# freewym/espresso

Hardware: AMD Instinct MI355X
Metric: audio-hours/sec training (LibriSpeech Conformer-12 + CTC) (higher is better)
Workload: dtype bf16; 1 GPU; LibriSpeech 960h Conformer-12 + CTC update step, <=26000 frames & <=24 utts per GPU, V=5004, on-GPU fbank+CMVN+SpecAugment, dropout 0.1, clip 2.0, Adam; parallelism=dp1

## Files before the change

espresso_amd/csrc/conv_igemm.hip:

```cpp
#include <hip/hip_runtime.h>

#include "gemm_common.h"

namespace {

typedef const __attribute__((address_space(1))) void* gptr_t;
typedef __attribute__((address_space(3))) void* lptr_t;

struct ConvGatherArgs {
  const bf16_t* src;
  const bf16_t* W;
  bf16_t* out;
  const float* bias;
  double* stats;
  const bf16_t* zero;
  int RB, RT, RF;
  int ST, SF, SC;
  int at, af;
  int ntaps;
  int bt[9], bf[9], koff[9];
  int N;
  long ldw;
  int OT, OF, ot_mul, ot_add, of_mul, of_add;
};

template <int BN_>
__global__ __launch_bounds__(256, 2) void conv_gather_kernel(const ConvGatherArgs a) {
  constexpr int BM_ = 128, NST = 2;
  constexpr int NJ = BN_ / 32;
  constexpr int A_BYTES = BM_ * ROW_BYTES, STAGE = A_BYTES + BN_ * ROW_BYTES;
  constexpr int NA = BM_ / 32, NB = BN_ / 32;
  extern __shared__ __attribute__((aligned(16))) char dsm[];
  const int tid = threadIdx.x, lane = tid & 63, wave = tid >> 6;
  const int wm = wave >> 1, wcol = (wave & 1) * (BN_ / 2);
  const uint32_t M = (uint32_t)a.RB * a.RT * a.RF;
  const uint32_t m0 = blockIdx.x * BM_;
  const int cpt = a.SC / BK;
  const int nk = a.ntaps * cpt;

  int rowb[NA], rowt[NA], rowf[NA];
  int cs[NA];
#pragma unroll
  for (int i = 0; i < NA; ++i) {
    const int r = (wave + 4 * i) * 8 + (lane >> 3);
    cs[i] = (lane & 7) ^ (r & 7) ^ ((r >> 4) & 7);
    const uint32_t p = m0 + r;
    if (p < M) {
      const uint32_t q = p / (uint32_t)a.RF, b = q / (uint32_t)a.RT;
      const int rf = (int)(p - q * a.RF), rt = (int)(q - b * a.RT);
      rowb[i] = (int)b * a.ST;
      rowt[i] = rt * a.at;
      rowf[i] = rf * a.af;
    } else {
      rowb[i] = -1;
      rowt[i] = rowf[i] = 0;
    }
  }
  const bf16_t* bp[NB];
#pragma unroll
  for (int i = 0; i < NB; ++i) {
    const int r = (wave + 4 * i) * 8 + (lane >> 3);
    const int c = (lane & 7) ^ (r & 7) ^ ((r >> 4) & 7);
    bp[i] = a.W + (long)min(r, a.N - 1) * a.ldw + c * 8;
  }
  auto issue = [&](int stage, int kt) {
    const int tap = kt / cpt, chunk = kt - tap * cpt;
    const int dt = a.bt[tap], df = a.bf[tap];
    const long ko = a.koff[tap] + chunk * BK;
    char* base = dsm + stage * STAGE + wave * 1024;
#pragma unroll
    for (int i = 0; i < NA; ++i) {
      const int st = rowt[i] + dt, sf = rowf[i] + df;
      const bool ok = rowb[i] >= 0 && (unsigned)st < (unsigned)a.ST && (unsigned)sf < (unsigned)a.SF;
      const bf16_t* s = ok ? a.src + (((long)(rowb[i] + st)) * a.SF + sf) * a.SC + chunk * BK + cs[i] * 8 : a.zero + cs[i] * 8;
      __builtin_amdgcn_global_load_lds((gptr_t)s, (lptr_t)(base + i * 4096), 16, 0, 0);
    }
#pragma unroll
    for (int i = 0; i < NB; ++i)
      __builtin_amdgcn_global_load_lds((gptr_t)(bp[i] + ko), (lptr_t)(base + A_BYTES + i * 4096), 16, 0, 0);
  };

  f32x4_t acc[4][NJ];
#pragma unroll
  for (int i = 0; i < 4; ++i)
#pragma unroll
    for (int j = 0; j < NJ; ++j) acc[i][j] = (f32x4_t){0.f, 0.f, 0.f, 0.f};
  uint32_t a_off[2][4], b_off[2][NJ];
#pragma unroll
  for (int ks = 0; ks < 2; ++ks) {
#pragma unroll
    for (int i = 0; i < 4; ++i) a_off[ks][i] = lds_off(wm * 64 + i * 16 + (lane & 15), ks * 4 + (lane >> 4));
#pragma unroll
    for (int j = 0; j < NJ; ++j) b_off[ks][j] = A_BYTES + lds_off(wcol + j * 16 + (lane & 15), ks * 4 + (lane >> 4));
  }

  if (nk > 0) issue(0, 0);
  int stage = 0;
  for (int kt = 0; kt < nk; ++kt) {
    asm volatile("s_waitcnt vmcnt(0)" ::: "memory");
    __builtin_amdgcn_s_barrier();
    if (kt + 1 < nk) issue(stage ^ 1, kt + 1);
    const char* st = dsm + stage * STAGE;
#pragma unroll
    for (int ks = 0; ks < 2; ++ks) {
      bf16x8_t af[4], bfr[NJ];
#pragma unroll
      for (int i = 0; i < 4; ++i) af[i] = *reinterpret_cast<const bf16x8_t*>(st + a_off[ks][i]);
#pragma unroll
      for (int j = 0; j < NJ; ++j) bfr[j] = *reinterpret_cast<const bf16x8_t*>(st + b_off[ks][j]);
#pragma unroll
      for (int i = 0; i < 4; ++i)
#pragma unroll
        for (int j = 0; j < NJ; ++j)
          acc[i][j] = __builtin_amdgcn_mfma_f32_16x16x32_bf16(
              __builtin_bit_cast(__attribute__((ext_vector_type(8))) __bf16, af[i]),
              __builtin_bit_cast(__attribute__((ext_vector_type(8))) __bf16, bfr[j]), acc[i][j], 0, 0, 0);
    }
    stage ^= 1;
  }

  constexpr int CG = BN_ / 8;
  constexpr int RL = 256 / CG;
  float* sC = reinterpret_cast<float*>(dsm);
  const int cg = tid % CG, rlane = tid / CG;
  float bias8[8], s8[8], q8[8];
#pragma unroll
  for (int e = 0; e < 8; ++e) {
    bias8[e] = a.bias ? a.bias[cg * 8 + e] : 0.f;
    s8[e] = q8[e] = 0.f;
  }
#pragma unroll 1
  for (int half = 0; half < 2; ++half) {
    __syncthreads();
    if (wm == half) {
#pragma unroll
      for (int i = 0; i < 4; ++i)
#pragma unroll
        for (int j = 0; j < NJ; ++j)
#pragma unroll
          for (int r = 0; r < 4; ++r) sC[(i * 16 + (lane >> 4) * 4 + r) * BN_ + wcol + j * 16 + (lane & 15)] = acc[i][j][r];
    }
    __syncthreads();
#pragma unroll 1
    for (int pass = 0; pass < 64 / RL; ++pass) {
      const int rl = pass * RL + rlane;
      const uint32_t p = m0 + half * 64 + rl;
      if (p < M) {
        const uint32_t q = p / (uint32_t)a.RF, b = q / (uint32_t)a.RT;
        const int rf = (int)(p - q * a.RF), rt = (int)(q - b * a.RT);
        const long orow = ((long)b * a.OT + (long)rt * a.ot_mul + a.ot_add) * a.OF + (long)rf * a.of_mul + a.of_add;
        const float4 x0 = *reinterpret_cast<const float4*>(sC + rl * BN_ + cg * 8);
        const float4 x1 = *reinterpret_cast<const float4*>(sC + rl * BN_ + cg * 8 + 4);
        float v[8] = {x0.x, x0.y, x0.z, x0.w, x1.x, x1.y, x1.z, x1.w};
#pragma unroll
        for (int e = 0; e < 8; ++e) v[e] += bias8[e];
        uint4 u;
        u.x = pack_bf2(v[0], v[1]); u.y = pack_bf2(v[2], v[3]); u.z = pack_bf2(v[4], v[5]); u.w = pack_bf2(v[6], v[7]);
        *reinterpret_cast<uint4*>(a.out + orow * a.N + cg * 8) = u;
        if (a.stats) {
          const uint32_t w[4] = {u.x, u.y, u.z, u.w};
#pragma unroll
          for (int e = 0; e < 4; ++e) {
            const float lo = __uint_as_float(w[e] << 16), hi = __uint_as_float(w[e] & 0xffff0000u);
            s8[2 * e] += lo; q8[2 * e] += lo * lo;
            s8[2 * e + 1] += hi; q8[2 * e + 1] += hi * hi;
          }
        }
      }
    }
  }
  if (a.stats) {
    __syncthreads();
    float* red = reinterpret_cast<float*>(dsm);
#pragma unroll
    for (int e = 0; e < 8; ++e) {
      red[(rlane * 2 + 0) * BN_ + cg * 8 + e] = s8[e];
      red[(rlane * 2 + 1) * BN_ + cg * 8 + e] = q8[e];
    }
    __syncthreads();
    if (tid < 2 * BN_) {
      const int which = tid / BN_, c = tid - which * BN_;
      float t = 0.f;
      for (int r = 0; r < RL; ++r) t += red[(r * 2 + which) * BN_ + c];
      atomicAdd(a.stats + which * a.N + c, (double)t);
    }
  }
}

const bf16_t* zero_line(hipStream_t stream) {
  static bf16_t* z = nullptr;
  if (!z) {
    if (hipMalloc(&z, 256) != hipSuccess) return nullptr;
    if (hipMemsetAsync(z, 0, 256, stream) != hipSuccess) return nullptr;
    hipStreamSynchronize(stream);
  }
  return z;
}

template <int BN_>
int launch_gather(const ConvGatherArgs& a, hipStream_t stream) {
  constexpr int bytes = 2 * (128 + BN_) * ROW_BYTES;
  static bool attr_ok = hipFuncSetAttribute(reinterpret_cast<const void*>(&conv_gather_kernel<BN_>),
                                            hipFuncAttributeMaxDynamicSharedMemorySize, bytes) == hipSuccess;
  if (!attr_ok) return -1;
  const long M = (long)a.RB * a.RT * a.RF;
  if (M <= 0) return 0;
  if (M >= (1L << 31) - 128) return -1;
  hipLaunchKernelGGL((conv_gather_kernel<BN_>), dim3((unsigned)((M + 127) / 128)), dim3(256), bytes, stream, a);
  return EA_CHECK_LAUNCH();
}


struct ConvWgradArgs {
  const bf16_t* X;
  const bf16_t* dZ;
  float* slab;
  const bf16_t* zero;
  int RB, RT, RF, ST, SF, Cin, Cout;
  int at, af, ntaps;
  int bt[9], bf[9];
  int chunks_per_wg;
  int ablate;
};

__device__ __forceinline__ int tr_sw(int r) { return (r & 3) ^ ((r >> 3) & 1); }
__device__ __forceinline__ void ds_read_tr16_x8(const uint32_t (&ad)[8], uint2 (&o)[8]) {
  asm volatile(
      "ds_read_b64_tr_b16 %0, %8\n\tds_read_b64_tr_b16 %1, %9\n\tds_read_b64_tr_b16 %2, %10\n\tds_read_b64_tr_b16 %3, %11\n\t"
      "ds_read_b64_tr_b16 %4, %12\n\tds_read_b64_tr_b16 %5, %13\n\tds_read_b64_tr_b16 %6, %14\n\tds_read_b64_tr_b16 %7, %15\n\t"
      "s_waitcnt lgkmcnt(0)"
      : "=&v"(o[0]), "=&v"(o[1]), "=&v"(o[2]), "=&v"(o[3]), "=&v"(o[4]), "=&v"(o[5]), "=&v"(o[6]), "=&v"(o[7])
      : "v"(ad[0]), "v"(ad[1]), "v"(ad[2]), "v"(ad[3]), "v"(ad[4]), "v"(ad[5]), "v"(ad[6]), "v"(ad[7])
      : "memory");
}

template <int DEPTH, int NT>
__global__ __launch_bounds__(256, NT == 9 ? 2 : 4) void conv_wgrad_kernel(const ConvWgradArgs a) {
  constexpr int TILE = 64 * ROW_BYTES;
  constexpr int NBUF = DEPTH == 1 ? 2 : 4;
  static_assert(DEPTH >= 1 && DEPTH <= 3 && (NT == 9 || NT == 3), "ring of two / four X tiles");
  const int tap0 = NT == 9 ? 0 : (int)(blockIdx.z % 3) * 3;
  const int zsplit = NT == 9 ? (int)blockIdx.z : (int)(blockIdx.z / 3);
  __shared__ __attribute__((aligned(16))) char lds[(2 + NBUF) * TILE];
  const int tid = threadIdx.x, lane = tid & 63, wave = tid >> 6;
  const int wr = wave >> 1, wc = wave & 1;
  const int co0 = blockIdx.x * 64, ci0 = blockIdx.y * 64;
  const long M = (long)a.RB * a.RT * a.RF;
  const long chunk0 = (long)zsplit * a.chunks_per_wg;
  long nch = (M + 63) / 64 - chunk0;
  if (nch > a.chunks_per_wg) nch = a.chunks_per_wg;
  if (nch < 0) nch = 0;

  f32x4_t acc[NT][2][2];
#pragma unroll
  for (int t = 0; t < NT; ++t)
#pragma unroll
    for (int i = 0; i < 2; ++i)
#pragma unroll
      for (int j = 0; j < 2; ++j) acc[t][i][j] = (f32x4_t){0.f, 0.f, 0.f, 0.f};

  int rr[2], cs[2];
#pragma unroll
  for (int i = 0; i < 2; ++i) {
    rr[i] = (wave + 4 * i) * 8 + (lane >> 3);
    cs[i] = (lane & 7) ^ (tr_sw(rr[i]) << 1);
  }
  int rowb[2], rowt[2], rowf[2];
  long rowp[2];
  auto decode = [&](long ch) {
#pragma unroll
    for (int i = 0; i < 2; ++i) {
      const long p = (chunk0 + ch) * 64 + rr[i];
      rowp[i] = p;
      if (p < M) {
        const uint32_t q = (uint32_t)p / (uint32_t)a.RF, b = q / (uint32_t)a.RT;
        rowb[i] = (int)b * a.ST;
        rowt[i] = (int)(q - b * a.RT) * a.at;
        rowf[i] = (int)((uint32_t)p - q * a.RF) * a.af;
      } else {
        rowb[i] = -1;
        rowt[i] = rowf[i] = 0;
      }
    }
  };
  auto issue_A = [&](int abuf) {
#pragma unroll
    for (int i = 0; i < 2; ++i) {
      const bf16_t* s = rowb[i] >= 0 ? a.dZ + rowp[i] * a.Cout + co0 + cs[i] * 8 : a.zero + cs[i] * 8;
      __builtin_amdgcn_global_load_lds((gptr_t)s, (lptr_t)(lds + abuf * TILE + (wave + 4 * i) * 1024), 16, 0, 0);
    }
  };
  auto issue_B = [&](int buf, int tap) {
#pragma unroll
    for (int i = 0; i < 2; ++i) {
      const int st = rowt[i] + a.bt[tap0 + tap], sf = rowf[i] + a.bf[tap0 + tap];
      const bool ok = rowb[i] >= 0 && (unsigned)st < (unsigned)a.ST && (unsigned)sf < (unsigned)a.SF;
      const bf16_t* s = ok ? a.X + (((long)(rowb[i] + st)) * a.SF + sf) * a.Cin + ci0 + cs[i] * 8 : a.zero + cs[i] * 8;
      __builtin_amdgcn_global_load_lds((gptr_t)s, (lptr_t)(lds + (2 + buf) * TILE + (wave + 4 * i) * 1024), 16, 0, 0);
    }
  };
  const uint32_t lds0 = (uint32_t)(uintptr_t)lds;
  auto read_frags = [&](int tile_off, int c0, uint4 (&fr)[2][2]) {
    const int g = lane >> 4, i = lane & 15;
    uint32_t ad[8];
    uint2 o[8];
#pragma unroll
    for (int ks = 0; ks < 2; ++ks)
#pragma unroll
      for (int t = 0; t < 2; ++t)
#pragma unroll
        for (int h = 0; h < 2; ++h) {
          const int r = ks * 32 + 8 * g + (i >> 2) + 4 * h;
          const int chunk = (c0 >> 4) + t;
          ad[(ks * 2 + t) * 2 + h] = lds0 + tile_off + r * ROW_BYTES + ((chunk ^ tr_sw(r)) << 5) + (i & 3) * 8;
        }
    ds_read_tr16_x8(ad, o);
#pragma unroll
    for (int ks = 0; ks < 2; ++ks)
#pragma unroll
      for (int t = 0; t < 2; ++t) fr[ks][t] = make_uint4(o[(ks * 2 + t) * 2].x, o[(ks * 2 + t) * 2].y, o[(ks * 2 + t) * 2 + 1].x, o[(ks * 2 + t) * 2 + 1].y);
  };

  const int nsteps = (int)nch * NT;
  int is = 0, itap = 0;
  long ich = 0;
  auto issue_next = [&]() {
    if (is >= nsteps) return;
    if (!(a.ablate & 2) || is < DEPTH) {
      if (itap == 0) {
        decode(ich);
        issue_A((int)(ich & 1));
      }
      issue_B(is & (NBUF - 1), itap);
    }
    ++is;
    if (++itap == NT) { itap = 0; ++ich; }
  };
#pragma unroll
  for (int d = 0; d < DEPTH; ++d) issue_next();
  uint4 fa[2][2];
  long ch = 0;
  int tap = 0;
  for (int s = 0; s < nsteps; ++s) {
    const int tap1 = tap + 1 == NT ? 0 : tap + 1, tap2 = tap1 + 1 == NT ? 0 : tap1 + 1;
    int pend = 0;
    if (DEPTH >= 2 && s + 1 < nsteps) pend += 2 + (tap1 == 0 ? 2 : 0);
    if (DEPTH >= 3 && s + 2 < nsteps) pend += 2 + (tap2 == 0 ? 2 : 0);
    if (pend >= 8) asm volatile("s_waitcnt vmcnt(8)" ::: "memory");
    else if (pend == 6) asm volatile("s_waitcnt vmcnt(6)" ::: "memory");
    else if (pend == 4) asm volatile("s_waitcnt vmcnt(4)" ::: "memory");
    else if (pend == 2) asm volatile("s_waitcnt vmcnt(2)" ::: "memory");
    else asm volatile("s_waitcnt vmcnt(0)" ::: "memory");
    if (!(a.ablate & 8)) __builtin_amdgcn_s_barrier();
    uint4 fb[2][2];
    if (!(a.ablate & 4) || s == 0) {
      if (tap == 0) read_frags((int)(ch & 1) * TILE, wr * 32, fa);
      read_frags((2 + (s & (NBUF - 1))) * TILE, wc * 32, fb);
    } else {
      fb[0][0] = fb[0][1] = fb[1][0] = fb[1][1] = fa[0][0];
    }
    __builtin_amdgcn_sched_barrier(0);
    issue_next();
    if (!(a.ablate & 1)) {
#pragma unroll
    for (int t = 0; t < NT; ++t) {
      if (t == tap) {
#pragma unroll
        for (int ks = 0; ks < 2; ++ks)
#pragma unroll
          for (int i = 0; i < 2; ++i)
#pragma unroll
            for (int j = 0; j < 2; ++j)
              acc[t][i][j] = __builtin_amdgcn_mfma_f32_16x16x32_bf16(
                  __builtin_bit_cast(__attribute__((ext_vector_type(8))) __bf16, fa[ks][i]),
                  __builtin_bit_cast(__attribute__((ext_vector_type(8))) __bf16, fb[ks][j]), acc[t][i][j], 0, 0, 0);
      }
    }
    } else {
      acc[0][0][0][0] += __uint_as_float(fb[0][0].x) + __uint_as_float(fb[1][1].y);
    }
    tap = tap1;
    if (tap1 == 0) ++ch;
  }

  float* out = a.slab + (long)zsplit * a.Cout * a.ntaps * a.Cin;
#pragma unroll
  for (int t = 0; t < NT; ++t) {
    {
#pragma unroll
      for (int i = 0; i < 2; ++i)
#pragma unroll
        for (int j = 0; j < 2; ++j)
#pragma unroll
          for (int r = 0; r < 4; ++r) {
            const int co = co0 + wr * 32 + i * 16 + (lane >> 4) * 4 + r, ci = ci0 + wc * 32 + j * 16 + (lane & 15);
            out[((long)co * a.ntaps + tap0 + t) * a.Cin + ci] = acc[t][i][j][r];
          }
    }
  }
}

__global__ __launch_bounds__(256) void conv_wgrad_reduce_kernel(const float* __restrict__ slab, float* __restrict__ dW, long n, int nsplit,
                                                                int cin = 0) {
  const int zper = (nsplit + gridDim.y - 1) / gridDim.y;
  const int z0 = blockIdx.y * zper, z1 = min(nsplit, z0 + zper);
  const long i = ((long)blockIdx.x * 256 + threadIdx.x) * 4;
  if (i >= n || z0 >= z1) return;
  float4 s = *reinterpret_cast<const float4*>(slab + (long)z0 * n + i);
  for (int z = z0 + 1; z < z1; ++z) {
    const float4 x = *reinterpret_cast<const float4*>(slab + (long)z * n + i);
    s.x += x.x; s.y += x.y; s.z += x.z; s.w += x.w;
  }
  if (cin > 0) {
    const long ct = i / cin;
    const int ci = (int)(i - ct * cin), tap = (int)(ct % 9);
    const long co = ct / 9;
    float* d = dW + (co * cin + ci) * 9 + tap;
    const float v[4] = {s.x, s.y, s.z, s.w};
#pragma unroll
    for (int e = 0; e < 4; ++e) {
      if (gridDim.y == 1) d[9 * e] += v[e];
      else atomicAdd(d + 9 * e, v[e]);
    }
    return;
  }
  if (gridDim.y == 1) {
    float4 d = *reinterpret_cast<const float4*>(dW + i);
    d.x += s.x; d.y += s.y; d.z += s.z; d.w += s.w;
    *reinterpret_cast<float4*>(dW + i) = d;
  } else {
    atomicAdd(dW + i, s.x); atomicAdd(dW + i + 1, s.y); atomicAdd(dW + i + 2, s.z); atomicAdd(dW + i + 3, s.w);
  }
}

static int wgrad_split(long M, int Cin, int Cout) {
  const long chunks = (M + 63) / 64;
  const int blocks = (Cin / 64) * (Cout / 64);
  static const long target = [] { const char* e = getenv("EA_CONV_WGRAD_WGS"); const long v = e ? atol(e) : 0; return v > 0 ? v : 256L; }();
  long nsplit = (target + blocks - 1) / blocks;
  if (nsplit > chunks / 8) nsplit = chunks / 8;
  if (nsplit < 1) nsplit = 1;
  return (int)nsplit;
}

}

extern "C" int ea_conv3x3_fwd(const void* X, const void* W, const float* bias, void* Z, double* stats, int B, int T, int F,
                              int Cin, int Cout, int sy, int sx, hipStream_t stream) {
  if (B <= 0 || T <= 0 || F <= 0) return 0;
  if (Cin % 64 || (Cout != 64 && Cout != 128) || sy < 1 || sx < 1) return -2;
  ConvGatherArgs a;
  a.src = (const bf16_t*)X; a.W = (const bf16_t*)W; a.out = (bf16_t*)Z; a.bias = bias; a.stats = stats;
  a.zero = zero_line(stream);
  if (!a.zero) return -1;
  const int To = (T - 1) / sy + 1, Fo = (F - 1) / sx + 1;
  a.RB = B; a.RT = To; a.RF = Fo;
  a.ST = T; a.SF = F; a.SC = Cin;
  a.at = sy; a.af = sx;
  a.ntaps = 9;
  for (int ky = 0; ky < 3; ++ky)
    for (int kx = 0; kx < 3; ++kx) {
      const int t = ky * 3 + kx;
      a.bt[t] = ky - 1; a.bf[t] = kx - 1; a.koff[t] = t * Cin;
    }
  a.N = Cout; a.ldw = 9L * Cin;
  a.OT = To; a.OF = Fo; a.ot_mul = 1; a.ot_add = 0; a.of_mul = 1; a.of_add = 0;
  return Cout == 128 ? launch_gather<128>(a, stream) : launch_gather<64>(a, stream);
}

extern "C" int ea_conv3x3_dgrad(const void* dZ, const void* Wd, void* dX, int B, int T, int F, int Cin, int Cout, int sy, int sx,
                                hipStream_t stream) {
  if (B <= 0 || T <= 0 || F <= 0) return 0;
  if (Cout % 64 || (Cin != 64 && Cin != 128) || sy < 1 || sx < 1 || sy > 2 || sx > 2) return -2;
  const int To = (T - 1) / sy + 1, Fo = (F - 1) / sx + 1;
  const bf16_t* zero = zero_line(stream);
  if (!zero) return -1;
  for (int pt = 0; pt < sy; ++pt)
    for (int pf = 0; pf < sx; ++pf) {
      ConvGatherArgs a;
      a.src = (const bf16_t*)dZ; a.W = (const bf16_t*)Wd; a.out = (bf16_t*)dX; a.bias = nullptr; a.stats = nullptr; a.zero = zero;
      a.RB = B; a.RT = (T - pt + sy - 1) / sy; a.RF = (F - pf + sx - 1) / sx;
      a.ST = To; a.SF = Fo; a.SC = Cout;
      a.at = 1; a.af = 1;
      a.ntaps = 0;
      for (int ky = 0; ky < 3; ++ky) {
        if ((pt + 1 - ky) % sy) continue;
        for (int kx = 0; kx < 3; ++kx) {
          if ((pf + 1 - kx) % sx) continue;
          const int t = a.ntaps++;
          a.bt[t] = (pt + 1 - ky) / sy; a.bf[t] = (pf + 1 - kx) / sx; a.koff[t] = (ky * 3 + kx) * Cout;
        }
      }
      a.N = Cin; a.ldw = 9L * Cout;
      a.OT = T; a.OF = F; a.ot_mul = sy; a.ot_add = pt; a.of_mul = sx; a.of_add = pf;
      if (a.RT <= 0 || a.RF <= 0) continue;
      if (a.ntaps == 0) return -2;
      const int rc = Cin == 128 ? launch_gather<128>(a, stream) : launch_gather<64>(a, stream);
      if (rc) return rc;
    }
  return 0;
}

extern "C" long ea_conv3x3_wgrad_workspace_bytes(int B, int T, int F, int Cin, int Cout, int sy, int sx) {
  const int To = (T - 1) / sy + 1, Fo = (F - 1) / sx + 1;
  return (long)wgrad_split((long)B * To * Fo, Cin, Cout) * Cout * 9 * Cin * (long)sizeof(float);
}

static int conv3x3_wgrad_impl(const void* X, const void* dZ, float* dW, void* workspace, int B, int T, int F, int Cin, int Cout,
                              int sy, int sx, int param_layout, hipStream_t stream);
extern "C" int ea_conv3x3_wgrad(const void* X, const void* dZ, float* dW, void* workspace, int B, int T, int F, int Cin, int Cout,
                                int sy, int sx, hipStream_t stream) {
  return conv3x3_wgrad_impl(X, dZ, dW, workspace, B, T, F, Cin, Cout, sy, sx, 0, stream);
}
extern "C" int ea_conv3x3_wgrad_param_layout(const void* X, const void* dZ, float* dW, void* workspace, int B, int T, int F, int Cin,
                                             int Cout, int sy, int sx, hipStream_t stream) {
  return conv3x3_wgrad_impl(X, dZ, dW, workspace, B, T, F, Cin, Cout, sy, sx, 1, stream);
}
static int conv3x3_wgrad_impl(const void* X, const void* dZ, float* dW, void* workspace, int B, int T, int F, int Cin, int Cout,
                              int sy, int sx, int param_layout, hipStream_t stream) {
  if (B <= 0 || T <= 0 || F <= 0) return 0;
  if (Cin % 64 || Cout % 64 || sy < 1 || sx < 1 || !workspace) return -2;
  ConvWgradArgs a;
  a.X = (const bf16_t*)X; a.dZ = (const bf16_t*)dZ; a.slab = (float*)workspace;
  a.zero = zero_line(stream);
  if (!a.zero) return -1;
  const int To = (T - 1) / sy + 1, Fo = (F - 1) / sx + 1;
  a.RB = B; a.RT = To; a.RF = Fo; a.ST = T; a.SF = F; a.Cin = Cin; a.Cout = Cout;
  a.at = sy; a.af = sx; a.ntaps = 9;
  for (int ky = 0; ky < 3; ++ky)
    for (int kx = 0; kx < 3; ++kx) { a.bt[ky * 3 + kx] = ky - 1; a.bf[ky * 3 + kx] = kx - 1; }
  const long M = (long)B * To * Fo;
  if (M >= (1L << 31) - 128) return -2;
  const int nsplit = wgrad_split(M, Cin, Cout);
  const long chunks = (M + 63) / 64;
  a.chunks_per_wg = (int)((chunks + nsplit - 1) / nsplit);
  static const int ablate = [] { const char* e = getenv("EA_CONVW_ABLATE"); return e ? atoi(e) : 0; }();
  a.ablate = ablate;
  static const int depth_env = [] { const char* e = getenv("EA_CONV_WGRAD_DEPTH"); return e ? atoi(e) : 0; }();
  const int depth = depth_env ? depth_env : (Cout <= 64 ? 3 : 1);
  static const int taps_env = [] { const char* e = getenv("EA_CONV_WGRAD_TAPS"); return e ? atoi(e) : 0; }();
  const int taps = taps_env == 3 || taps_env == 9 ? taps_env : 3;
  if (taps == 3) {
    hipLaunchKernelGGL((conv_wgrad_kernel<1, 3>), dim3(Cout / 64, Cin / 64, nsplit * 3), dim3(256), 0, stream, a);
  } else if (depth == 1) hipLaunchKernelGGL((conv_wgrad_kernel<1, 9>), dim3(Cout / 64, Cin / 64, nsplit), dim3(256), 0, stream, a);
  else if (depth == 2) hipLaunchKernelGGL((conv_wgrad_kernel<2, 9>), dim3(Cout / 64, Cin / 64, nsplit), dim3(256), 0, stream, a);
  else hipLaunchKernelGGL((conv_wgrad_kernel<3, 9>), dim3(Cout / 64, Cin / 64, nsplit), dim3(256), 0, stream, a);
  const long n = (long)Cout * 9 * Cin;
  const long blocks = (n / 4 + 255) / 256;
  int zg = (int)(1024 / blocks);
  if (zg > nsplit / 4) zg = nsplit / 4;
  if (zg < 1) zg = 1;
  hipLaunchKernelGGL(conv_wgrad_reduce_kernel, dim3((unsigned)blocks, zg), dim3(256), 0, stream, (const float*)workspace, dW, n, nsplit,
                     param_layout ? Cin : 0);
  return EA_CHECK_LAUNCH();
}
```

espresso_amd/csrc/convmodule.hip:

```cpp
#include "common.h"
#include "espresso_amd.h"

namespace {

constexpr int KMAX = 31;

__device__ __forceinline__ float sigmoid_f(float x) { return __builtin_amdgcn_rcpf(1.f + __expf(-x)); }

constexpr int CT = 64, TTILE = 64, TPT = TTILE / 4;

template <int KW>
__global__ __launch_bounds__(256) void glu_dwconv_fwd_kernel(const bf16_t* __restrict__ Y,
                                                             const float* __restrict__ w,
                                                             bf16_t* __restrict__ U, bf16_t* __restrict__ Z,
                                                             double* __restrict__ stats, int T, int C) {
  constexpr int PAD = (KW - 1) / 2, ROWS = TTILE + KW - 1;
  __shared__ __attribute__((aligned(16))) float su[ROWS][CT];
  __shared__ float sred[2][4][CT];
  const int c0 = blockIdx.x * CT, t0 = blockIdx.y * TTILE, b = blockIdx.z;
  const long rowbase = (long)b * T;
  if ((C & 7) == 0 && c0 + CT <= C) {
    bf16_t (*sub)[CT] = reinterpret_cast<bf16_t (*)[CT]>(&su[0][0]);
    bf16_t (*sz)[CT] = reinterpret_cast<bf16_t (*)[CT]>(&su[0][0]) + ROWS;
    constexpr int NCH = (ROWS * (CT / 8) + 255) / 256;
// ... 19 lines not shown
        const int tin = t0 - PAD + row;
        const uint32_t aw[4] = {va[k].x, va[k].y, va[k].z, va[k].w}, gw[4] = {vg[k].x, vg[k].y, vg[k].z, vg[k].w};
        uint32_t pk[4];
#pragma unroll
        for (int e = 0; e < 4; ++e)
          pk[e] = pack_bf2(__uint_as_float(aw[e] << 16) * sigmoid_f(__uint_as_float(gw[e] << 16)),
                           __uint_as_float(aw[e] & 0xffff0000u) * sigmoid_f(__uint_as_float(gw[e] & 0xffff0000u)));
        const bool inside = tin >= 0 && tin < T;
        const uint4 u4 = inside ? make_uint4(pk[0], pk[1], pk[2], pk[3]) : make_uint4(0, 0, 0, 0);
        if (inside && row >= PAD && row < PAD + TTILE) *reinterpret_cast<uint4*>(U + (rowbase + tin) * C + c0 + c8) = u4;
        *reinterpret_cast<uint4*>(&sub[row][c8]) = u4;
      }
    }
    __syncthreads();
    float acc[TPT];
#pragma unroll
    for (int j = 0; j < TPT; ++j) acc[j] = 0.f;
#pragma unroll
    for (int r = 0; r < TPT + KW - 1; ++r) {
      const float x = bf2f(sub[grp * TPT + r][cl]);
#pragma unroll
      for (int j = 0; j < TPT; ++j)
        if (r - j >= 0 && r - j < KW) acc[j] += wk[r - j] * x;
    }
    float s = 0.f, q = 0.f;
#pragma unroll
    for (int j = 0; j < TPT; ++j) {
      const int tout = t0 + grp * TPT + j;
      const bf16_t zb = f2bf(acc[j]);
      sz[grp * TPT + j][cl] = zb;
      if (tout < T) {
        const float z = bf2f(zb);
        s += z;
        q += z * z;
      }
    }
    if (stats) {
      sred[0][grp][cl] = s;
      sred[1][grp][cl] = q;
    }
    __syncthreads();
#pragma unroll
    for (int k = 0; k < 2; ++k) {
      const int i = threadIdx.x + 256 * k;
      const int r = i >> 3, c8 = (i & 7) * 8;
      if (t0 + r < T) *reinterpret_cast<uint4*>(Z + (rowbase + t0 + r) * C + c0 + c8) = *reinterpret_cast<const uint4*>(&sz[r][c8]);
    }
    if (stats && threadIdx.x < CT) {
      const int x = threadIdx.x;
      atomicAdd(stats + c0 + x, (double)(sred[0][0][x] + sred[0][1][x] + sred[0][2][x] + sred[0][3][x]));
      atomicAdd(stats + C + c0 + x, (double)(sred[1][0][x] + sred[1][1][x] + sred[1][2][x] + sred[1][3][x]));
    }
    return;
  }
  const bool vec = (C & 7) == 0;
  for (int i = threadIdx.x; i < ROWS * (CT / 8); i += 256) {
    const int row = i / (CT / 8), c8 = (i % (CT / 8)) * 8;
    const int tin = t0 - PAD + row;
    float u[8];
#pragma unroll
    for (int e = 0; e < 8; ++e) u[e] = 0.f;
    if (tin >= 0 && tin < T && c0 + c8 < C) {
      const bf16_t* yr = Y + (rowbase + tin) * (2L * C) + c0 + c8;
      uint32_t pk[4] = {0, 0, 0, 0};
      if (vec && c0 + c8 + 8 <= C) {
        const uint4 av = *reinterpret_cast<const uint4*>(yr);
        const uint4 gv = *reinterpret_cast<const uint4*>(yr + C);
        const uint32_t aw[4] = {av.x, av.y, av.z, av.w}, gw[4] = {gv.x, gv.y, gv.z, gv.w};
#pragma unroll
        for (int e = 0; e < 4; ++e)
          pk[e] = pack_bf2(__uint_as_float(aw[e] << 16) * sigmoid_f(__uint_as_float(gw[e] << 16)),
                           __uint_as_float(aw[e] & 0xffff0000u) * sigmoid_f(__uint_as_float(gw[e] & 0xffff0000u)));
        if (row >= PAD && row < PAD + TTILE)
          *reinterpret_cast<uint4*>(U + (rowbase + tin) * C + c0 + c8) = make_uint4(pk[0], pk[1], pk[2], pk[3]);
      } else {
        for (int e = 0; e < 8; ++e) {
          if (c0 + c8 + e >= C) break;
          const bf16_t ub = f2bf(bf2f(yr[e]) * sigmoid_f(bf2f(yr[C + e])));
          if (row >= PAD && row < PAD + TTILE) U[(rowbase + tin) * C + c0 + c8 + e] = ub;
          pk[e >> 1] |= (uint32_t)ub << (16 * (e & 1));
        }
      }
#pragma unroll
      for (int e = 0; e < 4; ++e) {
        u[2 * e] = __uint_as_float(pk[e] << 16);
        u[2 * e + 1] = __uint_as_float(pk[e] & 0xffff0000u);
      }
    }
    *reinterpret_cast<float4*>(&su[row][c8]) = make_float4(u[0], u[1], u[2], u[3]);
    *reinterpret_cast<float4*>(&su[row][c8 + 4]) = make_float4(u[4], u[5], u[6], u[7]);
  }
  const int cl = threadIdx.x & (CT - 1), grp = threadIdx.x >> 6;
  const int c = c0 + cl;
  float wk[KW];
#pragma unroll
  for (int k = 0; k < KW; ++k) wk[k] = c < C ? w[(long)c * KW + k] : 0.f;
  __syncthreads();
  float acc[TPT];
#pragma unroll
  for (int j = 0; j < TPT; ++j) acc[j] = 0.f;
#pragma unroll
  for (int r = 0; r < TPT + KW - 1; ++r) {
    const float x = su[grp * TPT + r][cl];
#pragma unroll
    for (int j = 0; j < TPT; ++j)
      if (r - j >= 0 && r - j < KW) acc[j] += wk[r - j] * x;
  }
  float s = 0.f, q = 0.f;
#pragma unroll
  for (int j = 0; j < TPT; ++j) {
    const int tout = t0 + grp * TPT + j;
    if (tout < T && c < C) {
      const bf16_t zb = f2bf(acc[j]);
      Z[(rowbase + tout) * C + c] = zb;
      const float z = bf2f(zb);
      s += z;
      q += z * z;
    }
  }
  if (stats) {
    sred[0][grp][cl] = s;
    sred[1][grp][cl] = q;
    __syncthreads();
    if (threadIdx.x < CT && c0 + threadIdx.x < C) {
      const int x = threadIdx.x;
      atomicAdd(stats + c0 + x, (double)(sred[0][0][x] + sred[0][1][x] + sred[0][2][x] + sred[0][3][x]));
      atomicAdd(stats + C + c0 + x, (double)(sred[1][0][x] + sred[1][1][x] + sred[1][2][x] + sred[1][3][x]));
    }
  }
}

__global__ void bn_finalize_kernel(const double* __restrict__ stats, float* __restrict__ mean_rstd,
                                   float* __restrict__ running_mean, float* __restrict__ running_var,
                                   int C, float n, float eps, float momentum) {
  const int c = blockIdx.x * blockDim.x + threadIdx.x;
  if (c >= C) return;
  const float mean = (float)(stats[c] / (double)n);
  float var = (float)(stats[C + c] / (double)n - (stats[c] / (double)n) * (stats[c] / (double)n));
  var = fmaxf(var, 0.f);
  mean_rstd[c] = mean;
  mean_rstd[C + c] = rsqrtf(var + eps);
  if (running_mean) {
    running_mean[c] = (1.f - momentum) * running_mean[c] + momentum * mean;
    const float unb = n > 1.f ? var * n / (n - 1.f) : var;
    running_var[c] = (1.f - momentum) * running_var[c] + momentum * unb;
  }
}
__global__ void bn_from_running_kernel(const float* __restrict__ running_mean, const float* __restrict__ running_var,
                                       float* __restrict__ mean_rstd, int C, float eps) {
  const int c = blockIdx.x * blockDim.x + threadIdx.x;
  if (c >= C) return;
  mean_rstd[c] = running_mean[c];
  mean_rstd[C + c] = rsqrtf(running_var[c] + eps);
}

__global__ __launch_bounds__(256) void bn_act_fwd_kernel(const bf16_t* __restrict__ Z, const float* __restrict__ mean_rstd,
                                                         const float* __restrict__ gamma, const float* __restrict__ beta,
                                                         bf16_t* __restrict__ Hout, long M, int C, int act) {
  const int nch = C >> 3;
  const long total = M * nch;
  const long stride = (long)gridDim.x * blockDim.x;
  const int ch = (int)(((long)blockIdx.x * blockDim.x + threadIdx.x) % nch);
  float sc[8], sh[8];
#pragma unroll
  for (int e = 0; e < 8; ++e) {
    const int c = ch * 8 + e;
    sc[e] = mean_rstd[C + c] * gamma[c];
    sh[e] = beta[c] - mean_rstd[c] * sc[e];
  }
  for (long i = (long)blockIdx.x * blockDim.x + threadIdx.x; i < total; i += stride) {
    const long m = i / nch;
    const uint4 u = *reinterpret_cast<const uint4*>(Z + m * C + ch * 8);
    const uint32_t wv[4] = {u.x, u.y, u.z, u.w};
    float o[8];
#pragma unroll
    for (int e = 0; e < 8; ++e) {
      const float z = (e & 1) ? __uint_as_float(wv[e >> 1] & 0xffff0000u) : __uint_as_float(wv[e >> 1] << 16);
      const float y = z * sc[e] + sh[e];
      o[e] = act == 2 ? silu_f(y) : (act == 1 ? fmaxf(y, 0.f) : y);
    }
    uint4 r;
    r.x = pack_bf2(o[0], o[1]); r.y = pack_bf2(o[2], o[3]); r.z = pack_bf2(o[4], o[5]); r.w = pack_bf2(o[6], o[7]);
    *reinterpret_cast<uint4*>(Hout + m * C + ch * 8) = r;
  }
}

__global__ __launch_bounds__(256) void bn_act_fwd_stats_kernel(const bf16_t* __restrict__ Z, const double* __restrict__ stats,
                                                               float* __restrict__ mean_rstd, float* __restrict__ running_mean,
                                                               float* __restrict__ running_var, const float* __restrict__ gamma,
                                                               const float* __restrict__ beta, bf16_t* __restrict__ Hout, long M,
                                                               int C, int act, float n, float eps, float momentum,
                                                               double* __restrict__ zero_next, int zero_n) {
  extern __shared__ float s_scsh[];
  const int nch = C >> 3;
  const long total = M * nch;
  const long stride = (long)gridDim.x * blockDim.x;
  const long gtid = (long)blockIdx.x * blockDim.x + threadIdx.x;
  const double inv_n = 1.0 / (double)n;
  for (int c = threadIdx.x; c < C; c += 256) {
    const double m1 = stats[c] * inv_n;
    const float mean = (float)m1;
    float var = (float)(stats[C + c] * inv_n - m1 * m1);
    var = fmaxf(var, 0.f);
    const float rstd = rsqrtf(var + eps);
    const float scv = rstd * gamma[c];
    s_scsh[c] = scv;
    s_scsh[C + c] = beta[c] - mean * scv;
    if (blockIdx.x == 0) {
      mean_rstd[c] = mean;
      mean_rstd[C + c] = rstd;
      if (running_mean) {
        running_mean[c] = (1.f - momentum) * running_mean[c] + momentum * mean;
        const float unb = n > 1.f ? var * n / (n - 1.f) : var;
        running_var[c] = (1.f - momentum) * running_var[c] + momentum * unb;
      }
    }
  }
  __syncthreads();
  const int ch = (int)(gtid % nch);
  float sc[8], sh[8];
#pragma unroll
  for (int e = 0; e < 8; ++e) {
    sc[e] = s_scsh[ch * 8 + e];
    sh[e] = s_scsh[C + ch * 8 + e];
  }
  for (long i = gtid; i < total; i += stride) {
    const long m = i / nch;
    const uint4 u = *reinterpret_cast<const uint4*>(Z + m * C + ch * 8);
    const uint32_t wv[4] = {u.x, u.y, u.z, u.w};
    float o[8];
#pragma unroll
    for (int e = 0; e < 8; ++e) {
      const float z = (e & 1) ? __uint_as_float(wv[e >> 1] & 0xffff0000u) : __uint_as_float(wv[e >> 1] << 16);
      const float y = z * sc[e] + sh[e];
      o[e] = act == 2 ? silu_f(y) : (act == 1 ? fmaxf(y, 0.f) : y);
    }
    uint4 r;
    r.x = pack_bf2(o[0], o[1]); r.y = pack_bf2(o[2], o[3]); r.z = pack_bf2(o[4], o[5]); r.w = pack_bf2(o[6], o[7]);
    *reinterpret_cast<uint4*>(Hout + m * C + ch * 8) = r;
  }
  if (zero_next)
    for (long i = gtid; i < zero_n; i += stride) zero_next[i] = 0.0;
}

__global__ __launch_bounds__(256) void bn_act_bwd_reduce_kernel(const bf16_t* __restrict__ Z, const bf16_t* __restrict__ dH,
                                                                const float* __restrict__ mean_rstd,
                                                                const float* __restrict__ gamma, const float* __restrict__ beta,
                                                                float* __restrict__ red, long M, int C, int act,
                                                                int rows_per_block, int TCH) {
  extern __shared__ float sm[];
  const int nch = C >> 3;
  const int cx = threadIdx.x % TCH, ry = threadIdx.x / TCH, lanes = 256 / TCH;
  const int ch = blockIdx.x * TCH + cx;
  const long r0 = (long)blockIdx.y * rows_per_block;
  const long r1 = min(M, r0 + rows_per_block);
  float sa[8], sb[8];
#pragma unroll
  for (int e = 0; e < 8; ++e) sa[e] = sb[e] = 0.f;
  if (ch < nch) {
    float mu[8], rs[8], ga[8], be[8];
#pragma unroll
    for (int e = 0; e < 8; ++e) {
      const int c = ch * 8 + e;
      mu[e] = mean_rstd[c]; rs[e] = mean_rstd[C + c]; ga[e] = gamma[c]; be[e] = beta[c];
    }
    auto accum = [&](const uint4& uz, const uint4& ud) {
      const uint32_t wz[4] = {uz.x, uz.y, uz.z, uz.w}, wd[4] = {ud.x, ud.y, ud.z, ud.w};
#pragma unroll
      for (int e = 0; e < 8; ++e) {
        const float z = (e & 1) ? __uint_as_float(wz[e >> 1] & 0xffff0000u) : __uint_as_float(wz[e >> 1] << 16);
        float d = (e & 1) ? __uint_as_float(wd[e >> 1] & 0xffff0000u) : __uint_as_float(wd[e >> 1] << 16);
        const float xh = (z - mu[e]) * rs[e];
        const float y = xh * ga[e] + be[e];
        d *= act == 2 ? dsilu_f(y) : (act == 1 ? (y > 0.f ? 1.f : 0.f) : 1.f);
        sa[e] += d;
        sb[e] += d * xh;
      }
    };
    constexpr int R = 4;
    long m = r0 + ry;
    for (; m + (long)(R - 1) * lanes < r1; m += (long)R * lanes) {
      uint4 uz[R], ud[R];
#pragma unroll
      for (int r = 0; r < R; ++r) {
        uz[r] = *reinterpret_cast<const uint4*>(Z + (m + (long)r * lanes) * C + ch * 8);
        ud[r] = *reinterpret_cast<const uint4*>(dH + (m + (long)r * lanes) * C + ch * 8);
      }
#pragma unroll
      for (int r = 0; r < R; ++r) accum(uz[r], ud[r]);
    }
    for (; m < r1; m += lanes) {
      const uint4 uz = *reinterpret_cast<const uint4*>(Z + m * C + ch * 8);
      const uint4 ud = *reinterpret_cast<const uint4*>(dH + m * C + ch * 8);
      accum(uz, ud);
    }
  }
  float* mine = sm + ((long)ry * TCH + cx) * 16;
#pragma unroll
  for (int e = 0; e < 8; ++e) { mine[e] = sa[e]; mine[8 + e] = sb[e]; }
  __syncthreads();
  for (int o = threadIdx.x; o < TCH * 16; o += 256) {
    const int cxo = o / 16, e = o % 16;
    const int cho = blockIdx.x * TCH + cxo;
    if (cho >= nch) continue;
    float a = 0.f;
    for (int r = 0; r < lanes; ++r) a += sm[((long)r * TCH + cxo) * 16 + e];
// ... 233 lines not shown
  const int cl = threadIdx.x & (CT - 1), grp = threadIdx.x >> 6;
  float acc[KG];
#pragma unroll
  for (int k = 0; k < KG; ++k) acc[k] = 0.f;
  const int tbeg = blockIdx.y * tiles_per_block * TTILE, tend = min(T, tbeg + tiles_per_block * TTILE);
  for (int t0 = tbeg; t0 < tend; t0 += TTILE) {
    __syncthreads();
    const bool c_ok = (C & 7) == 0;
    for (int i = threadIdx.x; i < (ROWS + KG) * (CT / 8); i += 256) {
      const int row = i / (CT / 8), c8 = (i % (CT / 8)) * 8;
      const int tin = t0 - PAD + row;
      float u[8];
#pragma unroll
      for (int e = 0; e < 8; ++e) u[e] = 0.f;
      if (row < ROWS && tin >= 0 && tin < T) {
        const bf16_t* src = U + (rowbase + tin) * C + c0 + c8;
        if (c_ok && c0 + c8 + 8 <= C) {
          const uint4 v = *reinterpret_cast<const uint4*>(src);
          const uint32_t w[4] = {v.x, v.y, v.z, v.w};
#pragma unroll
          for (int e = 0; e < 4; ++e) {
            u[2 * e] = __uint_as_float(w[e] << 16);
            u[2 * e + 1] = __uint_as_float(w[e] & 0xffff0000u);
          }
        } else {
          for (int e = 0; e < 8; ++e)
            if (c0 + c8 + e < C) u[e] = bf2f(src[e]);
        }
      }
      *reinterpret_cast<float4*>(&sU[row][c8]) = make_float4(u[0], u[1], u[2], u[3]);
      *reinterpret_cast<float4*>(&sU[row][c8 + 4]) = make_float4(u[4], u[5], u[6], u[7]);
    }
    for (int i = threadIdx.x; i < TTILE * (CT / 8); i += 256) {
      const int row = i / (CT / 8), c8 = (i % (CT / 8)) * 8;
      const int t = t0 + row;
      float d[8];
#pragma unroll
      for (int e = 0; e < 8; ++e) d[e] = 0.f;
      if (t < T) {
        const bf16_t* src = dZ + (rowbase + t) * C + c0 + c8;
        if (c_ok && c0 + c8 + 8 <= C) {
          const uint4 v = *reinterpret_cast<const uint4*>(src);
          const uint32_t w[4] = {v.x, v.y, v.z, v.w};
#pragma unroll
          for (int e = 0; e < 4; ++e) {
            d[2 * e] = __uint_as_float(w[e] << 16);
            d[2 * e + 1] = __uint_as_float(w[e] & 0xffff0000u);
          }
        } else {
          for (int e = 0; e < 8; ++e)
            if (c0 + c8 + e < C) d[e] = bf2f(src[e]);
        }
      }
      *reinterpret_cast<float4*>(&sD[row][c8]) = make_float4(d[0], d[1], d[2], d[3]);
      *reinterpret_cast<float4*>(&sD[row][c8 + 4]) = make_float4(d[4], d[5], d[6], d[7]);
    }
    __syncthreads();
    float x[KG];
#pragma unroll
    for (int kk = 0; kk < KG - 1; ++kk) x[kk + 1] = sU[grp * KG + kk][cl];
#pragma unroll
    for (int tt = 0; tt < TTILE; ++tt) {
#pragma unroll
      for (int kk = 0; kk < KG - 1; ++kk) x[kk] = x[kk + 1];
      x[KG - 1] = sU[tt + grp * KG + KG - 1][cl];
      const float d = sD[tt][cl];
#pragma unroll
      for (int kk = 0; kk < KG; ++kk) acc[kk] += d * x[kk];
    }
  }
  const int c = c0 + cl;
  if (c < C) {
    float* out = part + (((long)b * gridDim.y + blockIdx.y) * C + c) * KW;
#pragma unroll
    for (int kk = 0; kk < KG; ++kk)
      if (grp * KG + kk < KW) out[grp * KG + kk] = acc[kk];
  }
}
__global__ __launch_bounds__(256) void dwconv_weight_reduce_kernel(const float* __restrict__ part, float* __restrict__ dw, int nslab,
                                                                   int n) {
  const int i = blockIdx.x * 256 + threadIdx.x;
  if (i >= n) return;
  float a = 0.f;
  for (int s = blockIdx.y; s < nslab; s += gridDim.y) a += part[(long)s * n + i];
  if (gridDim.y == 1) dw[i] += a;
  else atomicAdd(dw + i, a);
}

static inline int egrid(long n) {
  long b = (n + 255) / 256;
  if (b > 8192) b = 8192;
  if (b < 1) b = 1;
  return (int)b;
}
static inline int egrid_ch(long n, int nch) {
  long b = egrid(n);
  while ((b * 256) % nch) ++b;
  return (int)b;
}

}

#define EA_KW_DISPATCH(KW, FN, ...)                  \
  switch (KW) {                                      \
    case 3: FN<3>(__VA_ARGS__); break;               \
    case 7: FN<7>(__VA_ARGS__); break;               \
    case 15: FN<15>(__VA_ARGS__); break;             \
    case 31: FN<31>(__VA_ARGS__); break;             \
    default: return -2;                              \
  }

template <int KW>
static void launch_glu_dwconv_fwd(dim3 grid, hipStream_t stream, const bf16_t* Y, const float* w, bf16_t* U, bf16_t* Z,
                                  double* stats, int T, int C) {
  hipLaunchKernelGGL((glu_dwconv_fwd_kernel<KW>), grid, dim3(256), 0, stream, Y, w, U, Z, stats, T, C);
}
template <int KW>
static void launch_glu_dwconv_bwd_data(dim3 grid, hipStream_t stream, const bf16_t* dZ, const bf16_t* Y, const float* w,
                                       bf16_t* dY, int T, int C) {
  hipLaunchKernelGGL((glu_dwconv_bwd_data_kernel<KW, false>), grid, dim3(256), 0, stream, dZ, Y, w, dY, T, C, BnBwdFuse{});
}
template <int KW>
static void launch_glu_dwconv_bwd_data_bn(dim3 grid, hipStream_t stream, const bf16_t* Y, const float* w, bf16_t* dY, int T, int C,
                                          BnBwdFuse fb) {
  hipLaunchKernelGGL((glu_dwconv_bwd_data_kernel<KW, true>), grid, dim3(256), 0, stream, (const bf16_t*)nullptr, Y, w, dY, T, C, fb);
}
template <int KW>
static void launch_dwconv_bwd_weight(dim3 grid, hipStream_t stream, const bf16_t* dZ, const bf16_t* U, float* dw, int T,
                                     int C, int tiles_per_block) {
  hipLaunchKernelGGL((dwconv_bwd_weight_kernel<KW>), grid, dim3(256), 0, stream, dZ, U, dw, T, C, tiles_per_block);
}

extern "C" int ea_glu_dwconv_fwd(const void* Y, const float* w, void* U, void* Z, double* stats, int B, int T,
                                 int C, int KW, hipStream_t stream) {
  if (B <= 0 || T <= 0) return 0;
  if (C % 2) return -2;
  dim3 grid((C + CT - 1) / CT, (T + TTILE - 1) / TTILE, B);
  EA_KW_DISPATCH(KW, launch_glu_dwconv_fwd, grid, stream, (const bf16_t*)Y, w, (bf16_t*)U, (bf16_t*)Z, stats, T, C);
  return EA_CHECK_LAUNCH();
}

extern "C" int ea_bn_finalize(const double* stats, float* mean_rstd, float* running_mean, float* running_var, int C,
                              float n, float eps, float momentum, hipStream_t stream) {
  hipLaunchKernelGGL(bn_finalize_kernel, dim3((C + 255) / 256), dim3(256), 0, stream, stats, mean_rstd, running_mean,
                     running_var, C, n, eps, momentum);
  return EA_CHECK_LAUNCH();
}
extern "C" int ea_bn_from_running(const float* running_mean, const float* running_var, float* mean_rstd, int C,
                                  float eps, hipStream_t stream) {
  hipLaunchKernelGGL(bn_from_running_kernel, dim3((C + 255) / 256), dim3(256), 0, stream, running_mean, running_var,
                     mean_rstd, C, eps);
  return EA_CHECK_LAUNCH();
}
extern "C" int ea_bn_act_fwd(const void* Z, const float* mean_rstd, const float* gamma, const float* beta, void* H,
                             long M, int C, int act, hipStream_t stream) {
  if (M <= 0) return 0;
  if (C % 8) return -2;
  hipLaunchKernelGGL(bn_act_fwd_kernel, dim3(egrid_ch(M * (C / 8), C / 8)), dim3(256), 0, stream, (const bf16_t*)Z, mean_rstd,
                     gamma, beta, (bf16_t*)H, M, C, act);
  return EA_CHECK_LAUNCH();
}
extern "C" int ea_bn_act_bwd(const void* Z, const void* dH, const float* mean_rstd, const float* gamma,
                             const float* beta, float* red , void* dZ, float* dgamma, float* dbeta,
                             long M, int C, int act, int training, hipStream_t stream);
extern "C" int ea_bn_act_fwd_train(const void* Z, const double* stats, float* mean_rstd, float* running_mean, float* running_var,
                                   const float* gamma, const float* beta, void* H, long M, int C, int act, float n, float eps,
                                   float momentum, double* zero_next, int zero_n, hipStream_t stream) {
  if (M <= 0) return 0;
  if (C % 8) return -2;
  hipLaunchKernelGGL(bn_act_fwd_stats_kernel, dim3(egrid_ch(M * (C / 8), C / 8)), dim3(256), (size_t)2 * C * sizeof(float), stream, (const bf16_t*)Z, stats,
                     mean_rstd, running_mean, running_var, gamma, beta, (bf16_t*)H, M, C, act, n, eps, momentum, zero_next, zero_n);
  return EA_CHECK_LAUNCH();
}

namespace {
__device__ __forceinline__ int c1_sw(int r) { return (r & 3) ^ ((r >> 3) & 1); }
__device__ __forceinline__ void c1_tr_read8(const uint32_t (&ad)[8], uint2 (&o)[8]) {
  asm volatile(
      "ds_read_b64_tr_b16 %0, %8\n\tds_read_b64_tr_b16 %1, %9\n\tds_read_b64_tr_b16 %2, %10\n\tds_read_b64_tr_b16 %3, %11\n\t"
      "ds_read_b64_tr_b16 %4, %12\n\tds_read_b64_tr_b16 %5, %13\n\tds_read_b64_tr_b16 %6, %14\n\tds_read_b64_tr_b16 %7, %15\n\t"
      "s_waitcnt lgkmcnt(0)"
      : "=&v"(o[0]), "=&v"(o[1]), "=&v"(o[2]), "=&v"(o[3]), "=&v"(o[4]), "=&v"(o[5]), "=&v"(o[6]), "=&v"(o[7])
      : "v"(ad[0]), "v"(ad[1]), "v"(ad[2]), "v"(ad[3]), "v"(ad[4]), "v"(ad[5]), "v"(ad[6]), "v"(ad[7])
      : "memory");
}
__global__ __launch_bounds__(256) void conv1_bn_bwd_wgrad_kernel(const float* __restrict__ X, const bf16_t* __restrict__ Z,
                                                                 const bf16_t* __restrict__ dH, const float* __restrict__ mean_rstd,
                                                                 const float* __restrict__ gamma, const float* __restrict__ beta,
                                                                 const float* __restrict__ red, float* __restrict__ dW,
                                                                 float* __restrict__ dbias, int T, int F, int To, int Fo, int CO,
                                                                 int sy, int sx, long npos, int act, float n) {
  __shared__ __attribute__((aligned(16))) char tile[4][32 * 128];
  __shared__ float sred[4][64][16];
  const int lane = threadIdx.x & 63, wave = threadIdx.x >> 6;
  const int li = lane & 15, g4 = lane >> 4;
  const float invn = n > 0.f ? 1.f / n : 0.f;
  const long nblk = (npos + 31) / 32;
  const long bmax = (npos - 1) / ((long)Fo * To);
  const uint32_t lds0 = (uint32_t)(uintptr_t)(&tile[wave][0]);
  for (int cs = 0; cs < CO; cs += 64) {
    const int c8 = lane & 7, prow = lane >> 3;
    float mu[8], rs[8], ga[8], be[8], r0[8], r1[8];
#pragma unroll
    for (int e = 0; e < 8; ++e) {
      const int c = cs + c8 * 8 + e;
      mu[e] = mean_rstd[c]; rs[e] = mean_rstd[CO + c]; ga[e] = gamma[c]; be[e] = beta[c];
      r0[e] = red[c] * invn; r1[e] = red[CO + c] * invn;
    }
    f32x4_t acc[4];
#pragma unroll
    for (int mt = 0; mt < 4; ++mt) acc[mt] = (f32x4_t){0.f, 0.f, 0.f, 0.f};
    for (long blk = (long)blockIdx.x * 4 + wave; blk < nblk; blk += (long)gridDim.x * 4) {
      const long pb = blk * 32;
      uint4 uz4[4], ud4[4];
#pragma unroll
      for (int it = 0; it < 4; ++it) {
        const long p = min(pb + prow + 8 * it, npos - 1);
        uz4[it] = *reinterpret_cast<const uint4*>(Z + p * CO + cs + c8 * 8);
        ud4[it] = *reinterpret_cast<const uint4*>(dH + p * CO + cs + c8 * 8);
      }
      int fo = (int)(pb % Fo), to = (int)((pb / Fo) % To);
      long b = pb / ((long)Fo * To);
      float xs[8];
      bool xv[8];
#pragma unroll
      for (int j = 0; j < 8; ++j) {
        const int k = 8 * g4 + j;
        int f = fo + k, t = to;
        long bb = b;
        while (f >= Fo) { f -= Fo; ++t; }
        while (t >= To) { t -= To; ++bb; }
        const int tap = li < 9 ? li : 0;
        const int ti = t * sy + tap / 3 - 1, fi = f * sx + tap % 3 - 1;
        xv[j] = pb + k < npos && li < 9 && ti >= 0 && ti < T && fi >= 0 && fi < F;
        const int tc = min(max(ti, 0), T - 1), fc = min(max(fi, 0), F - 1);
        const long bc = bb < bmax ? bb : bmax;
        xs[j] = X[(bc * T + tc) * F + fc];
      }
#pragma unroll
      for (int it = 0; it < 4; ++it) {
        const int r = prow + 8 * it;
        const long p = pb + r;
        uint4 o = make_uint4(0, 0, 0, 0);
        {
          const uint4 uz = uz4[it], ud = ud4[it];
          const uint32_t wz[4] = {uz.x, uz.y, uz.z, uz.w}, wd[4] = {ud.x, ud.y, ud.z, ud.w};
          float d[8];
#pragma unroll
          for (int e = 0; e < 8; ++e) {
            const float z = (e & 1) ? __uint_as_float(wz[e >> 1] & 0xffff0000u) : __uint_as_float(wz[e >> 1] << 16);
            float g = (e & 1) ? __uint_as_float(wd[e >> 1] & 0xffff0000u) : __uint_as_float(wd[e >> 1] << 16);
            const float xh = (z - mu[e]) * rs[e];
            const float y = xh * ga[e] + be[e];
            g *= act == 2 ? dsilu_f(y) : (act == 1 ? (y > 0.f ? 1.f : 0.f) : 1.f);
            d[e] = rs[e] * ga[e] * (g - r0[e] - xh * r1[e]);
          }
          o.x = pack_bf2(d[0], d[1]); o.y = pack_bf2(d[2], d[3]); o.z = pack_bf2(d[4], d[5]); o.w = pack_bf2(d[6], d[7]);
        }
        if (p >= npos) o = make_uint4(0, 0, 0, 0);
        *reinterpret_cast<uint4*>(&tile[wave][r * 128 + (((c8 >> 1) ^ c1_sw(r)) << 5) + (c8 & 1) * 16]) = o;
      }
      uint32_t bh[4], bl[4];
#pragma unroll
      for (int j = 0; j < 8; ++j) {
        const int k = 8 * g4 + j;
        float x = xv[j] ? xs[j] : 0.f;
        if (li == 9 && pb + k < npos) x = 1.f;
        const uint32_t hi = (uint32_t)f2bf(x);
        const uint32_t lo = (uint32_t)f2bf(x - __uint_as_float(hi << 16));
        if (j & 1) { bh[j >> 1] |= hi << 16; bl[j >> 1] |= lo << 16; }
        else { bh[j >> 1] = hi; bl[j >> 1] = lo; }
      }
      __builtin_amdgcn_fence(__ATOMIC_RELEASE, "wavefront");
      __builtin_amdgcn_wave_barrier();
      __builtin_amdgcn_fence(__ATOMIC_ACQUIRE, "wavefront");
      uint32_t ad[8];
      uint2 o8[8];
#pragma unroll
      for (int mt = 0; mt < 4; ++mt)
#pragma unroll
        for (int h = 0; h < 2; ++h) {
          const int r = 8 * g4 + 4 * h + (li >> 2);
          ad[mt * 2 + h] = lds0 + r * 128 + ((mt ^ c1_sw(r)) << 5) + (li & 3) * 8;
        }
      c1_tr_read8(ad, o8);
      const bf16x8_t vbh = __builtin_bit_cast(bf16x8_t, make_uint4(bh[0], bh[1], bh[2], bh[3]));
      const bf16x8_t vbl = __builtin_bit_cast(bf16x8_t, make_uint4(bl[0], bl[1], bl[2], bl[3]));
#pragma unroll
      for (int mt = 0; mt < 4; ++mt) {
        const bf16x8_t a8 = __builtin_bit_cast(bf16x8_t, make_uint4(o8[mt * 2].x, o8[mt * 2].y, o8[mt * 2 + 1].x, o8[mt * 2 + 1].y));
        acc[mt] = __builtin_amdgcn_mfma_f32_16x16x32_bf16(__builtin_bit_cast(__attribute__((ext_vector_type(8))) __bf16, a8),
                                                          __builtin_bit_cast(__attribute__((ext_vector_type(8))) __bf16, vbh), acc[mt], 0, 0, 0);
        acc[mt] = __builtin_amdgcn_mfma_f32_16x16x32_bf16(__builtin_bit_cast(__attribute__((ext_vector_type(8))) __bf16, a8),
                                                          __builtin_bit_cast(__attribute__((ext_vector_type(8))) __bf16, vbl), acc[mt], 0, 0, 0);
      }
      __builtin_amdgcn_wave_barrier();
    }
#pragma unroll
    for (int mt = 0; mt < 4; ++mt)
#pragma unroll
      for (int r = 0; r < 4; ++r) sred[wave][mt * 16 + g4 * 4 + r][li] = acc[mt][r];
    __syncthreads();
    for (int i = threadIdx.x; i < 64 * 10; i += 256) {
      const int c = i / 10, k = i % 10;
      const float a = sred[0][c][k] + sred[1][c][k] + sred[2][c][k] + sred[3][c][k];
      if (k < 9) atomicAdd(dW + (cs + c) * 9 + k, a);
// ... 127 lines not shown
```

espresso_amd/functional.py:

```python
import collections

import ctypes
import os

import torch

from . import kernels as K

_seed_state = {"base": 0x5EED, "counter": 0}


def set_dropout_seed(seed: int):
    _seed_state["base"] = int(seed) & 0xFFFFFFFF
    _seed_state["counter"] = 0


_seed_trace = None


class trace_dropout_seeds:

    def __enter__(self):
        global _seed_trace
        self.prev, self.entries = _seed_trace, []
# ... 503 lines not shown
                K.add2_strided(t1, C, t2, C, dqkv, 3 * C, M, C)
        else:
            K.add2_strided(t1, C, torch.zeros_like(t1), C, dqkv, 3 * C, M, C)
        dWqkv = _wgrad(dqkv, xn, M, 3 * C, C)
        dbqkv = K.colsum(dqkv, _zeros_f32(3 * C, x), M, 3 * C, 3 * C)
        dxn = _new((M, C), torch.bfloat16, x)
        K.gemm(dqkv, wqkv16, dxn, M, C, 3 * C, lda=3 * C, ldb=C, ldc=C, b_kstrided=True)
        if pre_ln:
            dg, db = _zeros_f32(C, x), _zeros_f32(C, x)
            dx = K.layernorm_bwd(x, dxn, ln_g, mean, rstd, dg, db, dx_add=dy)
        else:
            dg = db = None
            dx = K.scale_dropout(dxn, a=1.0, y=dy, b=1.0)
        return (dx, dg, db, dWqkv, dbqkv, dWo, dbo, du, dv, dWpos, None, None, None, dpe) + (None,) * 10


def relpos_mhsa(x, ln_g, ln_b, wqkv, bqkv, wo, bo, u, v, wpos, pe, key_len, attn_mask, B, T, H, p_attn=0.0, p_out=0.0,
                eps=1e-5, pre_ln=True, wqkv16=None, causal=False):
    return _RelPosMHSA.apply(
        x, ln_g, ln_b, wqkv, bqkv, wo, bo, u, v, wpos, wqkv16 if wqkv16 is not None else bf16_weight(wqkv),
        bf16_weight(wo), bf16_weight(wpos) if wpos is not None else None, pe, key_len, attn_mask, B, T, H, p_attn, p_out,
        eps, pre_ln, causal)


class _ConvModule(torch.autograd.Function):

    @staticmethod
    def forward(ctx, x, ln_g, ln_b, wpw1, wdw, bn_g, bn_b, wpw2, wpw1_16, wpw2_16, running_mean, running_var, B, T, KW,
                p_out, eps, bn_eps, bn_momentum, training):
        M, C = x.shape
        xn, mean, rstd = K.layernorm_fwd(x, ln_g, ln_b, eps)
        Y = _new((M, 2 * C), torch.bfloat16, x)
        K.gemm(xn, wpw1_16, Y, M, 2 * C, C, lda=C, ldb=C, ldc=2 * C)
        wdw2 = wdw.detach().reshape(C, KW).contiguous()
        stats = torch.zeros(2 * C, dtype=torch.float64, device=x.device) if training else None
        U, Zt = K.glu_dwconv_fwd(Y, wdw2, B, T, C, KW, stats)
        if training:
            mr = K.bn_finalize(stats, C, M, bn_eps, bn_momentum, running_mean, running_var)
        else:
            mr = K.bn_from_running(running_mean, running_var, bn_eps)
        Hh = K.bn_act_fwd(Zt, mr, bn_g, bn_b, "silu")
        so = _next_seed("conv.out", p_out) if p_out > 0 else 0
        y = _new((M, C), torch.bfloat16, x)
        K.gemm(Hh, wpw2_16, y, M, C, C, lda=C, ldb=C, ldc=C, drop_p=p_out, drop_seed=so, resid=x, ldr=C)
        ctx.save_for_backward(x, ln_g, mean, rstd, xn, Y, U, Zt, mr, Hh, bn_g, bn_b, wdw2, wpw1_16, wpw2_16)
        ctx.cfg = (B, T, KW, p_out, so, training)
        ctx.wdw_shape = wdw.shape
        return y

    @staticmethod
    def backward(ctx, dy):
        (x, ln_g, mean, rstd, xn, Y, U, Zt, mr, Hh, bn_g, bn_b, wdw2, wpw1_16, wpw2_16) = ctx.saved_tensors
        B, T, KW, p_out, so, training = ctx.cfg
        M, C = x.shape
        dy = dy.contiguous()
        g = K.scale_dropout(dy, a=1.0, drop_p=p_out, drop_seed=so) if p_out > 0 else dy
        dWpw2 = _wgrad(g, Hh, M, C, C)
        dH = _new((M, C), torch.bfloat16, x)
        K.gemm(g, wpw2_16, dH, M, C, C, lda=C, ldb=C, ldc=C, b_kstrided=True)
        dbn_g, dbn_b = _zeros_f32(C, x), _zeros_f32(C, x)
        dZ = K.bn_act_bwd(Zt, dH, mr, bn_g, bn_b, dbn_g, dbn_b, "silu", training)
        dwdw = _zeros_f32(C * KW, x)
        dY = K.glu_dwconv_bwd(dZ, Y, U, wdw2, dwdw, B, T, C, KW)
        dWpw1 = _wgrad(dY, xn, M, 2 * C, C)
        dxn = _new((M, C), torch.bfloat16, x)
        K.gemm(dY, wpw1_16, dxn, M, C, 2 * C, lda=2 * C, ldb=C, ldc=C, b_kstrided=True)
        dg, db = _zeros_f32(C, x), _zeros_f32(C, x)
        dx = K.layernorm_bwd(x, dxn, ln_g, mean, rstd, dg, db, dx_add=dy)
        return (dx, dg, db, dWpw1.view(2 * C, C, 1), dwdw.view(ctx.wdw_shape), dbn_g, dbn_b, dWpw2.view(C, C, 1)) + (None,) * 12


def conv_module(x, ln_g, ln_b, wpw1, wdw, bn_g, bn_b, wpw2, running_mean, running_var, B, T, p_out=0.0, eps=1e-5,
                bn_eps=1e-5, bn_momentum=0.1, training=True):
    C = x.shape[1]
    KW = wdw.shape[-1]
    return _ConvModule.apply(x, ln_g, ln_b, wpw1, wdw, bn_g, bn_b, wpw2, bf16_weight(wpw1).view(2 * C, C),
                             bf16_weight(wpw2).view(C, C), running_mean, running_var, B, T, KW, p_out, eps, bn_eps,
                             bn_momentum, training)


class _CTCLoss(torch.autograd.Function):

    @staticmethod
    def forward(ctx, logits, targets, in_len, tgt_len, B, T, blank, zero_infinity):
        M, V = logits.shape
        assert M == B * T
        if logits.stride(1) != 1:
            logits = logits.contiguous()
        Lmax = targets.shape[1]
        lprobs = K.log_softmax(logits, M, V, logits.stride(0))
        nll, ws = K.ctc_loss_fwd(lprobs, targets, in_len, tgt_len, B, T, V, Lmax, blank)
        ctx.save_for_backward(lprobs, ws, nll, targets, in_len, tgt_len)
        ctx.cfg = (B, T, V, Lmax, blank, zero_infinity, logits.dtype)
        ctx.mark_non_differentiable(lprobs)
        return nll, lprobs

    @staticmethod
    def backward(ctx, dnll, _dlp):
        lprobs, ws, nll, targets, in_len, tgt_len = ctx.saved_tensors
        B, T, V, Lmax, blank, zero_infinity, dt = ctx.cfg
        scale_dev = dnll.float().contiguous()
        bf = dt == torch.bfloat16
        ld = _pad8(V) if bf else V
        dl = K.ctc_loss_grad(lprobs, ws, nll, targets, in_len, tgt_len, B, T, V, Lmax, blank, ld_out=ld, grad_bf16=bf,
                             grad_scale=1.0, grad_scale_dev=scale_dev, zero_infinity=zero_infinity)
        return (dl if ld == V else dl[:, :V]), None, None, None, None, None, None, None


def ctc_loss(logits, targets, in_len, tgt_len, B, T, blank=0, zero_infinity=True):
    return _CTCLoss.apply(logits, targets, in_len, tgt_len, B, T, blank, zero_infinity)


class _LabelSmoothedCE(torch.autograd.Function):

    @staticmethod
    def forward(ctx, logits, target, pad_idx, eps, smoothing="uniform", prior=None, tgt_len=0):
        M, V = logits.shape
        if logits.stride(1) != 1:
            logits = logits.contiguous()
        out, _ = K.label_smoothed_ce(logits, logits.stride(0), target, M, V, pad_idx, eps, want_grad=False, smoothing=smoothing,
                                     prior=prior, tgt_len=tgt_len)
        ctx.save_for_backward(logits, target, prior)
        ctx.cfg = (pad_idx, eps, smoothing, tgt_len)
        return out[0], out[1]

    @staticmethod
    def backward(ctx, dloss, _dnll):
        logits, target, prior = ctx.saved_tensors
        pad_idx, eps, smoothing, tgt_len = ctx.cfg
        M, V = logits.shape
        bf = logits.dtype == torch.bfloat16
        _, dl = K.label_smoothed_ce(logits, logits.stride(0), target, M, V, pad_idx, eps, want_grad=True, grad_bf16=bf,
                                    grad_ld=_pad8(V) if bf else V, smoothing=smoothing, prior=prior, tgt_len=tgt_len)
        g = dl if dl.shape[1] == V else dl[:, :V]
        return g * dloss.to(g.dtype), None, None, None, None, None, None


def label_smoothed_ce(logits, target, pad_idx, eps, smoothing="uniform", prior=None, tgt_len=0):
    return _LabelSmoothedCE.apply(logits, target, pad_idx, eps, smoothing, prior, tgt_len)


_CONV_IGEMM = True


_CONV1_FUSED_BWD = True


def set_conv1_fused_backward(on: bool) -> bool:
    global _CONV1_FUSED_BWD
    old, _CONV1_FUSED_BWD = _CONV1_FUSED_BWD, bool(on)
    return old


def set_conv_implicit_gemm(on: bool):
    global _CONV_IGEMM
    _CONV_IGEMM = bool(on)


def _conv_igemm_ok(cin, cout, sy, sx):
    return _CONV_IGEMM and cin in (64, 128) and cout in (64, 128) and sy in (1, 2) and sx in (1, 2)


class _ConvSubsample(torch.autograd.Function):

    @staticmethod
    def forward(ctx, X, row_zero, strides, bufs, p_drop, training, bn_eps, bn_momentum, *params):
        B, T, F = X.shape
        L = len(params) // 4
        saved = []
        cfgs = []
        A = None
        Tc, Fc, Cc = T, F, 1
        for i in range(L):
            w, b, g, beta = params[4 * i: 4 * i + 4]
            rm, rv = bufs[2 * i], bufs[2 * i + 1]
            sy, sx = strides[i]
            Co = w.shape[0]
            To, Fo = (Tc - 1) // sy + 1, (Fc - 1) // sx + 1
            stats = _pool_zeros((2 * Co,), torch.float64, X.device) if training else None
            if i == 0:
                assert w.shape[1] == 1 and tuple(w.shape[2:]) == (3, 3)
                Zi = K.conv1_fwd(X, w.detach().reshape(Co, 9).contiguous(), b, B, Tc, Fc, Co, sy, sx, stats)
                col, w16 = None, None
            elif _conv_igemm_ok(Cc, Co, sy, sx):
                w16 = K.cast_f32_to_bf16(w.detach().permute(0, 2, 3, 1).reshape(Co, 9 * Cc).contiguous())
                Zi = K.conv3x3_fwd(A, w16, b, B, Tc, Fc, Cc, Co, sy, sx, stats=stats)
                col = A
            else:
                col = K.im2col3x3(A, B, Tc, Fc, Cc, sy, sx)
                w16 = K.cast_f32_to_bf16(w.detach().permute(0, 2, 3, 1).reshape(Co, 9 * Cc).contiguous())
                Zi = _new((B * To * Fo, Co), torch.bfloat16, X)
                K.gemm(col, w16, Zi, B * To * Fo, Co, 9 * Cc, lda=9 * Cc, ldb=9 * Cc, ldc=Co, bias=b)
                if training:
                    K.colstats(Zi, stats)
            n = B * To * Fo
            mr = K.bn_finalize(stats, Co, n, bn_eps, bn_momentum, rm, rv) if training else K.bn_from_running(rm, rv, bn_eps)
            A = K.bn_act_fwd(Zi, mr, g, beta, "relu")
            saved += [Zi, mr, col, w16, g, beta]
            cfgs.append((Tc, Fc, Cc, To, Fo, Co, sy, sx))
            Tc, Fc, Cc = To, Fo, Co
        out = A.view(B * Tc, Fc * Cc)
        seed = _next_seed("subsample.out", p_drop) if (training and p_drop > 0) else 0
        if seed:
            out = K.scale_dropout(out, a=1.0, drop_p=p_drop, drop_seed=seed)
        if row_zero is not None:
            K.zero_rows(out, row_zero)
        ctx.save_for_backward(X, row_zero, *[t for t in saved if t is not None])
        ctx.layout = [[t is not None for t in saved[6 * i: 6 * i + 6]] for i in range(L)]
        ctx.cfg = (B, cfgs, p_drop, seed, training, [tuple(p.shape) for p in params[0::4]])
        ctx.igemm = [i > 0 and _conv_igemm_ok(cfgs[i][2], cfgs[i][5], cfgs[i][6], cfgs[i][7]) for i in range(L)]
        ctx.weights = [params[4 * i] for i in range(L)]
        ctx.params = list(params)
        return out

    @staticmethod
    def backward(ctx, dout):
        X, row_zero, *flat = ctx.saved_tensors
        B, cfgs, p_drop, seed, training, wshapes = ctx.cfg
        L = len(cfgs)
        it = iter(flat)
        per = []
        for i in range(L):
            per.append([next(it) if has else None for has in ctx.layout[i]])
        dout = dout.contiguous()
        if seed:
            dout = K.scale_dropout(dout, a=1.0, drop_p=p_drop, drop_seed=seed)
        elif row_zero is not None:
            dout = dout.clone()
        if row_zero is not None:
            K.zero_rows(dout, row_zero)
        grads = [None] * (4 * L)
        Tc, Fc, Cc, To, Fo, Co, sy, sx = cfgs[-1]
        dA = dout.view(B * To * Fo, Co)
        cur = torch.cuda.current_stream(X.device)
        side = _side_stream(X.device)
        keep = []
        for i in range(L - 1, -1, -1):
            Zi, mr, col, w16, g, beta = per[i]
            Tc, Fc, Cc, To, Fo, Co, sy, sx = cfgs[i]
            pw, pb, pg, pbe = ctx.params[4 * i: 4 * i + 4]
            sg, sbe = (_grad_sink(pg, Co), _grad_sink(pbe, Co)) if training else (None, None)
            if sg is not None and sbe is not None:
                dg, dbeta = sg, sbe
            else:
                sg = sbe = None
                dg, dbeta = _zeros_f32(Co, X), _zeros_f32(Co, X)
            if i == 0 and Co % 64 == 0 and _CONV1_FUSED_BWD:
                sW, sb = _grad_sink(pw, Co * 9), _grad_sink(pb, Co)
                if sW is not None and sb is not None:
                    db, dW = sb, sW
                else:
                    sW = None
                    db, dW = _zeros_f32(Co, X), _zeros_f32(Co * 9, X)
                K.conv1_bn_bwd(X, Zi, dA, mr, g, beta, dg, dbeta, dW, db, B, Tc, Fc, Co, sy, sx, "relu", training)
                if sW is None:
                    grads[0], grads[1] = dW.view(wshapes[0]), db
                if sg is None:
                    grads[2], grads[3] = dg, dbeta
                continue
            dZ = K.bn_act_bwd(Zi, dA, mr, g, beta, dg, dbeta, "relu", training)
            keep.append(dZ)
            n = B * To * Fo
            db = _zeros_f32(Co, X)
            if i == 0:
                dW = _zeros_f32(Co * 9, X)
                side.wait_stream(cur)
                with torch.cuda.stream(side):
                    K.conv1_wgrad(X, dZ, dW, db, B, Tc, Fc, Co, sy, sx)
                grads[0] = dW.view(wshapes[0])
            elif ctx.igemm[i]:
                sW = _grad_sink(pw, Co * 9 * Cc)
                side.wait_stream(cur)
                if sW is not None:
                    with torch.cuda.stream(side):
                        K.conv3x3_wgrad(col, dZ, sW, B, Tc, Fc, Cc, Co, sy, sx, param_layout=True)
                else:
                    dWp = _zeros_f32(Co * 9 * Cc, X).view(Co, 9 * Cc)
                    with torch.cuda.stream(side):
                        K.conv3x3_wgrad(col, dZ, dWp, B, Tc, Fc, Cc, Co, sy, sx)
                    grads[4 * i] = dWp.view(Co, 3, 3, Cc).permute(0, 3, 1, 2)
                if not training:
                    db = g.detach() * mr[1] * dbeta
                elif _grad_sink(pb, Co) is not None:
                    db = None
                wd16 = K.cast_f32_to_bf16(ctx.weights[i].detach().permute(1, 2, 3, 0).reshape(Cc, 9 * Co).contiguous())
                dA = K.conv3x3_dgrad(dZ, wd16, B, Tc, Fc, Cc, Co, sy, sx)
            else:
                dWp = torch.empty((Co, 9 * Cc), dtype=torch.float32, device=X.device)
                side.wait_stream(cur)
                with torch.cuda.stream(side):
                    _wgrad(dZ, col, n, Co, 9 * Cc, out=dWp)
                    K.colsum(dZ, db, n, Co, Co)
                grads[4 * i] = dWp.view(Co, 3, 3, Cc).permute(0, 3, 1, 2)
                dcol = _new((n, 9 * Cc), torch.bfloat16, X)
                K.gemm(dZ, w16, dcol, n, 9 * Cc, Co, lda=Co, ldb=9 * Cc, ldc=9 * Cc, b_kstrided=True)
                dA = K.col2im3x3(dcol, B, Tc, Fc, Cc, sy, sx)
            grads[4 * i + 1] = db
            if sg is None:
                grads[4 * i + 2] = dg
                grads[4 * i + 3] = dbeta
        cur.wait_stream(side)
        del keep
        return (None,) * 8 + tuple(grads)


def conv_subsample(X, row_zero, strides, params, bufs, p_drop=0.0, training=True, bn_eps=1e-5, bn_momentum=0.1):
    return _ConvSubsample.apply(X, row_zero, tuple(strides), list(bufs), p_drop, training, bn_eps, bn_momentum, *params)


_grad_ready_callback = None


def set_grad_ready_callback(fn):
    global _grad_ready_callback
    _grad_ready_callback = fn


def _ptr(t):
    return None if t is None else t.data_ptr()


class _LayerBinding:

    def __init__(self, m, kind="conformer"):
        import ctypes

        from ._lib import EaConformerLayer

        self.keep = []
        self.kind = kind
        L = EaConformerLayer()

        def w16(p, shape=None):
            t = bf16_weight(p)
            t = t.reshape(shape) if shape is not None else t
            self.keep.append(t)
            return t.data_ptr()

        def grad(p):
            if p.grad is None:
                p.grad = torch.zeros_like(p)
            return p.grad.data_ptr()

        def ffn(dst, gdst, f):
            dst.ln_g, dst.ln_b = _ptr(f.layer_norm.weight), _ptr(f.layer_norm.bias)
            dst.w1, dst.b1, dst.w2, dst.b2 = w16(f.w_1.weight), _ptr(f.w_1.bias), w16(f.w_2.weight), _ptr(f.w_2.bias)
            gdst.ln_g, gdst.ln_b = grad(f.layer_norm.weight), grad(f.layer_norm.bias)
            gdst.w1, gdst.b1, gdst.w2, gdst.b2 = grad(f.w_1.weight), grad(f.w_1.bias), grad(f.w_2.weight), grad(f.w_2.bias)

        if kind == "conformer":
            ffn(L.ffn1, L.grads.ffn1, m.ffn1)
            ffn(L.ffn2, L.grads.ffn2, m.ffn2)
            Cm, Fm = m.embed_dim, m.ffn1.w_1.weight.shape[0]
            self.wt = torch.empty(4 * Cm * Fm + 7 * Cm * Cm, dtype=torch.bfloat16, device=m.ffn1.w_1.weight.device)
        else:
            f1, gf = L.ffn1, L.grads.ffn1
            f1.ln_g, f1.ln_b = _ptr(m.final_layer_norm.weight), _ptr(m.final_layer_norm.bias)
            f1.w1, f1.b1, f1.w2, f1.b2 = w16(m.fc1.weight), _ptr(m.fc1.bias), w16(m.fc2.weight), _ptr(m.fc2.bias)
            gf.ln_g, gf.ln_b = grad(m.final_layer_norm.weight), grad(m.final_layer_norm.bias)
            gf.w1, gf.b1, gf.w2, gf.b2 = grad(m.fc1.weight), grad(m.fc1.bias), grad(m.fc2.weight), grad(m.fc2.bias)
            Cm, Fm = m.embed_dim, m.fc1.weight.shape[0]
            self.wt = torch.empty(2 * Cm * Fm + 4 * Cm * Cm, dtype=torch.bfloat16, device=m.fc1.weight.device)
        L.wt = self.wt.data_ptr()
        a = m.self_attn
        qw, kw, vw = a.q_proj.weight, a.k_proj.weight, a.v_proj.weight
        qb, kb, vb = a.q_proj.bias, a.k_proj.bias, a.v_proj.bias
        for p in (qw, kw, vw, qb, kb, vb):
            grad(p)
        fused16 = getattr(qw, "_ea_fused_qkv", None)
        n = qw.numel()
        grads_contig = (qw.grad is not None and kw.grad is not None and vw.grad is not None
                        and kw.grad.data_ptr() == qw.grad.data_ptr() + 4 * n and vw.grad.data_ptr() == kw.grad.data_ptr() + 4 * n)
        if fused16 is not None and grads_contig:
            wqkv16, self.split_w = fused16, None
            gw = qw.grad.data_ptr()
        else:
            wqkv16 = torch.cat([bf16_weight(qw), bf16_weight(kw), bf16_weight(vw)], 0)
            gbuf = torch.zeros(3 * qw.shape[0], qw.shape[1], dtype=torch.float32, device=qw.device)
            self.split_w = (gbuf, (qw, kw, vw))
            gw = gbuf.data_ptr()
        self.keep.append(wqkv16)
        nb = qb.numel()
        bias_contig = (kb.data_ptr() == qb.data_ptr() + 4 * nb and vb.data_ptr() == kb.data_ptr() + 4 * nb
                       and qb.grad is not None and kb.grad is not None and vb.grad is not None
                       and kb.grad.data_ptr() == qb.grad.data_ptr() + 4 * nb and vb.grad.data_ptr() == kb.grad.data_ptr() + 4 * nb)
        if bias_contig:
            self.split_b = None
            bq_ptr, gb_ptr = qb.data_ptr(), qb.grad.data_ptr()
        else:
            bq = torch.cat([qb.detach(), kb.detach(), vb.detach()], 0)
            gb = torch.zeros_like(bq)
            self.split_b = (gb, (qb, kb, vb))
            self.keep += [bq, gb]
            bq_ptr, gb_ptr = bq.data_ptr(), gb.data_ptr()
        self.cacheable = self.split_w is None and self.split_b is None
        self.key = (qw.data_ptr(), qw.grad.data_ptr() if qw.grad is not None else 0)
        A, GA = L.attn, L.grads.attn
        A.ln_g, A.ln_b = _ptr(m.self_attn_layer_norm.weight), _ptr(m.self_attn_layer_norm.bias)
        A.wqkv, A.bqkv, A.wo, A.bo = wqkv16.data_ptr(), bq_ptr, w16(a.out_proj.weight), _ptr(a.out_proj.bias)
        GA.ln_g, GA.ln_b = grad(m.self_attn_layer_norm.weight), grad(m.self_attn_layer_norm.bias)
        GA.wqkv, GA.bqkv, GA.wo, GA.bo = gw, gb_ptr, grad(a.out_proj.weight), grad(a.out_proj.bias)
        if a.pos_proj is not None:
            A.pos_u, A.pos_v, A.wpos = _ptr(a.pos_bias_u), _ptr(a.pos_bias_v), w16(a.pos_proj.weight)
            GA.pos_u, GA.pos_v, GA.wpos = grad(a.pos_bias_u), grad(a.pos_bias_v), grad(a.pos_proj.weight)
        for p in (qw, kw, vw, qb, kb, vb):
            grad(p)
        self.saved_buf, self.saved_busy = None, False
        self.L = L
        if kind != "conformer":
            mods = [a.q_proj, a.k_proj, a.v_proj, a.out_proj, m.self_attn_layer_norm, m.fc1, m.fc2, m.final_layer_norm]
            self.params = [p for mod in mods for p in mod.parameters()]
            if a.pos_proj is not None:
                self.params += [a.pos_bias_u, a.pos_bias_v, a.pos_proj.weight]
            return
        cm = m.conv_module
        Cc, GC = L.conv, L.grads.conv
        Cdim = m.embed_dim
        Cc.ln_g, Cc.ln_b = _ptr(cm.layer_norm.weight), _ptr(cm.layer_norm.bias)
        Cc.pw1 = w16(cm.pointwise_conv1.weight, (2 * Cdim, Cdim))
        Cc.dw = _ptr(cm.depthwise_conv.weight)
        Cc.bn_g, Cc.bn_b = _ptr(cm.batch_norm.weight), _ptr(cm.batch_norm.bias)
        Cc.bn_rm, Cc.bn_rv = _ptr(cm.batch_norm.running_mean), _ptr(cm.batch_norm.running_var)
        Cc.pw2 = w16(cm.pointwise_conv2.weight, (Cdim, Cdim))
        GC.ln_g, GC.ln_b = grad(cm.layer_norm.weight), grad(cm.layer_norm.bias)
        GC.pw1, GC.dw = grad(cm.pointwise_conv1.weight), grad(cm.depthwise_conv.weight)
        GC.bn_g, GC.bn_b, GC.pw2 = grad(cm.batch_norm.weight), grad(cm.batch_norm.bias), grad(cm.pointwise_conv2.weight)
        L.final_ln_g, L.final_ln_b = _ptr(m.final_layer_norm.weight), _ptr(m.final_layer_norm.bias)
        L.grads.final_ln_g, L.grads.final_ln_b = grad(m.final_layer_norm.weight), grad(m.final_layer_norm.bias)
        self.L = L
        self.params = [p for p in m.parameters()]
        self.saved_buf, self.saved_busy = None, False

# ... 1172 lines not shown
```

espresso_amd/kernels.py:

```python
import ctypes
from typing import Optional

import torch

from . import _lib
from ._lib import EaGemmParams, check

ACT_NONE, ACT_RELU, ACT_SILU = 0, 1, 2
_ACT = {None: 0, "none": 0, "relu": 1, "silu": 2, "swish": 2}


def _stream():
    return ctypes.c_void_p(torch._C._cuda_getCurrentRawStream(torch._C._cuda_getDevice()))


def _p(t: Optional[torch.Tensor]):
    if t is None:
        return None
    if not t.is_cuda:
        raise RuntimeError("espresso_amd kernels need device tensors (no CPU path)")
    return ctypes.c_void_p(t.data_ptr())


def drop_params(p: float):
# ... 124 lines not shown
def cast_f32_to_bf16_rows(src, ld_dst):
    M, N = src.shape
    assert src.dtype == torch.float32 and src.stride(1) == 1 and ld_dst >= N
    dst = torch.empty(M, ld_dst, dtype=torch.bfloat16, device=src.device)
    check(_lib.lib().ea_cast_f32_to_bf16_rows(_p(src), src.stride(0), _p(dst), ld_dst, M, N, _stream()), "ea_cast_f32_to_bf16_rows")
    return dst if ld_dst == N else dst[:, :N]


def cast_bf16_to_f32(src, dst=None):
    if dst is None:
        dst = torch.empty(src.shape, dtype=torch.float32, device=src.device)
    check(_lib.lib().ea_cast_bf16_to_f32(_p(src), _p(dst), src.numel(), _stream()), "ea_cast_bf16_to_f32")
    return dst


def scale_dropout(x, a=1.0, y=None, b=0.0, drop_p=0.0, drop_seed=0, out=None):
    assert x.dtype == torch.bfloat16 and x.is_contiguous()
    if out is None:
        out = torch.empty_like(x)
    thr, scale = drop_params(drop_p)
    check(_lib.lib().ea_scale_dropout_bf16(_p(x), _p(y), _p(out), x.numel(), a, b, drop_seed, thr, scale, _stream()),
          "ea_scale_dropout_bf16")
    return out


def colsum(X, out, M, N, ld):
    assert X.dtype == torch.bfloat16 and out.dtype == torch.float32
    check(_lib.lib().ea_colsum_bf16(_p(X), _p(out), M, N, ld, _stream()), "ea_colsum_bf16")
    return out


def colsum_ptr(X_ptr: int, out, M, N, ld):
    check(_lib.lib().ea_colsum_bf16(ctypes.c_void_p(X_ptr), _p(out), M, N, ld, _stream()), "ea_colsum_bf16")
    return out


def zero_rows(x, row_zero):
    M, C = x.shape
    check(_lib.lib().ea_zero_rows_bf16(_p(x), _p(row_zero), M, C, _stream()), "ea_zero_rows_bf16")
    return x


def relpos_q_prep(qkv, ldq, u, v, M, C, scaling, want_qv=True):
    qu = torch.empty(M, C, dtype=torch.bfloat16, device=qkv.device)
    qv = torch.empty(M, C, dtype=torch.bfloat16, device=qkv.device) if want_qv else None
    check(_lib.lib().ea_relpos_q_prep(_p(qkv), ldq, _p(u), _p(v), _p(qu), _p(qv), M, C, scaling, _stream()),
          "ea_relpos_q_prep")
    return qu, qv


def relpos_softmax_fwd(ac, bd, key_len, attn_mask, H, B, T, S, ld_ac, ld_bd, ld_p, causal=False, drop_p=0.0,
                       drop_seed=0):
    P = torch.empty(H * B * T, ld_p, dtype=torch.bfloat16, device=ac.device)
    Pd = torch.empty_like(P) if drop_p > 0 else None
    thr, scale = drop_params(drop_p)
    check(
        _lib.lib().ea_relpos_softmax_fwd(_p(ac), _p(bd), _p(key_len), _p(attn_mask), _p(P), _p(Pd), H, B, T, S, ld_ac,
                                         ld_bd, ld_p, int(causal), drop_seed, thr, scale, _stream()),
        "ea_relpos_softmax_fwd",
    )
    return P, (Pd if Pd is not None else P)


def flash_attention_supported(dh, T, S, relpos):
    return bool(_lib.lib().ea_flash_attention_supported(dh, T, S, int(relpos)))


def flash_keep_bits_buffer(H, B, T, device):
    return torch.empty(int(_lib.lib().ea_flash_keep_bits_bytes(H, B, T)) // 2, dtype=torch.int16, device=device)


def flash_attention_fwd(qu, qv, k, v, pp, key_len, H, B, T, S, ldq, ldkv, ldpp=0, causal=False, drop_p=0.0, drop_seed=0,
                        want_lse=True, want_bits=False):
    dh = 64
    out = torch.empty(B * T, H * dh, dtype=torch.bfloat16, device=qu.device)
    lse = torch.empty(H * B, T, dtype=torch.float32, device=qu.device) if want_lse else None
    thr, scale = drop_params(drop_p)
    bits = None
    if want_bits and thr and qv is not None and T == S and not causal:
        bits = flash_keep_bits_buffer(H, B, T, qu.device)
    check(
        _lib.lib().ea_flash_attention_fwd(_p(qu), _p(qv), ldq, _p(k), _p(v), ldkv, _p(pp), ldpp, _p(key_len), _p(out),
                                          H * dh, _p(lse), H, B, T, S, dh, int(causal), drop_seed, thr, scale, _p(bits), _stream()),
        "ea_flash_attention_fwd",
    )
    return (out, lse, bits) if want_bits else (out, lse)


def flash_attention_bwd(qu, qv, k, v, pp, key_len, out, dout, lse, dk, dv, H, B, T, S, ldq, ldkv, lddkv, ldpp=0, causal=False,
                        scaling=1.0, drop_p=0.0, drop_seed=0, keep_bits=None, dq=None, lddq=0):
    dh = 64
    C = H * dh
    relpos = qv is not None
    t1 = torch.empty(B * T, C, dtype=torch.bfloat16, device=qu.device)
    t2 = torch.empty_like(t1) if relpos else None
    Rp = (2 * T - 1 + 7) // 8 * 8
    dBD = torch.empty(H * B * T, Rp, dtype=torch.bfloat16, device=qu.device) if relpos else None
    D = torch.empty(H * B, T, dtype=torch.float32, device=qu.device)
    thr, scale = drop_params(drop_p)
    check(
        _lib.lib().ea_flash_attention_bwd(_p(qu), _p(qv), ldq, _p(k), _p(v), ldkv, _p(pp), ldpp, _p(key_len), _p(out), _p(dout),
                                          C, _p(lse), _p(D), _p(t1), _p(t2), C, _p(dBD), Rp, _p(dk), _p(dv), lddkv, H, B, T, S,
                                          dh, int(causal), scaling, drop_seed, thr, scale, _p(keep_bits), _p(dq), lddq,
                                          _stream()),
        "ea_flash_attention_bwd",
    )
    return t1, t2, dBD


def relpos_softmax_bwd(P, dPd, H, B, T, S, ld_p, ld_dp, ld_bd, want_bd=True, drop_p=0.0, drop_seed=0):
    dAC = torch.empty(H * B * T, ld_p, dtype=torch.bfloat16, device=P.device)
    dBD = torch.empty(H * B * T, ld_bd, dtype=torch.bfloat16, device=P.device) if want_bd else None
    thr, scale = drop_params(drop_p)
    check(
        _lib.lib().ea_relpos_softmax_bwd(_p(P), _p(dPd), _p(dAC), _p(dBD), H, B, T, S, ld_p, ld_dp, ld_bd, drop_seed,
                                         thr, scale, _stream()),
        "ea_relpos_softmax_bwd",
    )
    return dAC, dBD


def add2_strided(a, lda, b, ldb, out, ldo, M, C, out_off=0):
    check(
        _lib.lib().ea_add2_strided_bf16(_p(a), lda, _p(b), ldb, ctypes.c_void_p(out.data_ptr() + 2 * out_off), ldo, M,
                                        C, _stream()),
        "ea_add2_strided_bf16",
    )
    return out


def glu_dwconv_fwd(Y, w, B, T, C, KW, stats):
    U = torch.empty(B * T, C, dtype=torch.bfloat16, device=Y.device)
    Z = torch.empty(B * T, C, dtype=torch.bfloat16, device=Y.device)
    check(_lib.lib().ea_glu_dwconv_fwd(_p(Y), _p(w), _p(U), _p(Z), _p(stats), B, T, C, KW, _stream()),
          "ea_glu_dwconv_fwd")
    return U, Z


def bn_finalize(stats, C, n, eps, momentum, running_mean=None, running_var=None):
    mean_rstd = torch.empty(2, C, dtype=torch.float32, device=stats.device)
    check(_lib.lib().ea_bn_finalize(_p(stats), _p(mean_rstd), _p(running_mean), _p(running_var), C, float(n), eps,
                                    momentum, _stream()), "ea_bn_finalize")
    return mean_rstd


def bn_from_running(running_mean, running_var, eps):
    C = running_mean.numel()
    mean_rstd = torch.empty(2, C, dtype=torch.float32, device=running_mean.device)
    check(_lib.lib().ea_bn_from_running(_p(running_mean), _p(running_var), _p(mean_rstd), C, eps, _stream()),
          "ea_bn_from_running")
    return mean_rstd


def bn_act_fwd(Z, mean_rstd, gamma, beta, act):
    M, C = Z.shape
    H = torch.empty_like(Z)
    check(_lib.lib().ea_bn_act_fwd(_p(Z), _p(mean_rstd), _p(gamma), _p(beta), _p(H), M, C, _ACT[act], _stream()),
          "ea_bn_act_fwd")
    return H


def conv1_bn_bwd(X, Z, dH, mean_rstd, gamma, beta, dgamma, dbeta, dW, dbias, B, T, F, CO, sy, sx, act, training=True):
    from . import functional as _F

    red = _F._pool_zeros((2, CO), torch.float32, Z.device)
    check(_lib.lib().ea_conv1_bn_bwd(_p(X), _p(Z), _p(dH), _p(mean_rstd), _p(gamma), _p(beta), _p(red), _p(dgamma), _p(dbeta), _p(dW),
                                     _p(dbias), B, T, F, CO, sy, sx, _ACT[act], int(training), _stream()), "ea_conv1_bn_bwd")


def bn_act_bwd(Z, dH, mean_rstd, gamma, beta, dgamma, dbeta, act, training=True):
    M, C = Z.shape
    from . import functional as _F

    red = _F._pool_zeros((2, C), torch.float32, Z.device)
    dZ = torch.empty_like(Z)
    check(
        _lib.lib().ea_bn_act_bwd(_p(Z), _p(dH), _p(mean_rstd), _p(gamma), _p(beta), _p(red), _p(dZ), _p(dgamma),
                                 _p(dbeta), M, C, _ACT[act], int(training), _stream()),
        "ea_bn_act_bwd",
    )
    return dZ


def glu_dwconv_bwd(dZ, Y, U, w, dw, B, T, C, KW):
    dY = torch.empty(B * T, 2 * C, dtype=torch.bfloat16, device=Y.device)
    ws = torch.empty(int(_lib.lib().ea_dwconv_wgrad_workspace_bytes(B, T, C, KW)), dtype=torch.uint8, device=Y.device)
    check(_lib.lib().ea_glu_dwconv_bwd(_p(dZ), _p(Y), _p(U), _p(w), _p(dY), _p(dw), _p(ws), B, T, C, KW, _stream()),
          "ea_glu_dwconv_bwd")
    return dY


def conv1_fwd(X, W, bias, B, T, F, CO, sy, sx, stats):
    To, Fo = (T - 1) // sy + 1, (F - 1) // sx + 1
    Z = torch.empty(B * To * Fo, CO, dtype=torch.bfloat16, device=X.device)
    check(_lib.lib().ea_conv1_fwd(_p(X), _p(W), _p(bias), _p(Z), _p(stats), B, T, F, CO, sy, sx, _stream()),
          "ea_conv1_fwd")
    return Z


def conv1_wgrad(X, dZ, dW, dbias, B, T, F, CO, sy, sx):
    check(_lib.lib().ea_conv1_wgrad(_p(X), _p(dZ), _p(dW), _p(dbias), B, T, F, CO, sy, sx, _stream()), "ea_conv1_wgrad")


def conv3x3_fwd(X, W16, bias, B, T, F, Cin, Cout, sy, sx, stats=None):
    To, Fo = (T - 1) // sy + 1, (F - 1) // sx + 1
    Z = torch.empty((B * To * Fo, Cout), dtype=torch.bfloat16, device=X.device)
    check(_lib.lib().ea_conv3x3_fwd(_p(X), _p(W16), _p(bias), _p(Z), _p(stats), B, T, F, Cin, Cout, sy, sx, _stream()), "ea_conv3x3_fwd")
    return Z


def conv3x3_dgrad(dZ, Wd16, B, T, F, Cin, Cout, sy, sx):
    dX = torch.empty((B * T * F, Cin), dtype=torch.bfloat16, device=dZ.device)
    check(_lib.lib().ea_conv3x3_dgrad(_p(dZ), _p(Wd16), _p(dX), B, T, F, Cin, Cout, sy, sx, _stream()), "ea_conv3x3_dgrad")
    return dX


def conv3x3_wgrad(X, dZ, dW, B, T, F, Cin, Cout, sy, sx, param_layout=False):
    lib = _lib.lib()
    nb = lib.ea_conv3x3_wgrad_workspace_bytes(B, T, F, Cin, Cout, sy, sx)
    ws = torch.empty(nb, dtype=torch.uint8, device=X.device)
    fn = lib.ea_conv3x3_wgrad_param_layout if param_layout else lib.ea_conv3x3_wgrad
    check(fn(_p(X), _p(dZ), _p(dW), _p(ws), B, T, F, Cin, Cout, sy, sx, _stream()), "ea_conv3x3_wgrad")
    return dW


def im2col3x3(A, B, T, F, C, sy, sx):
    To, Fo = (T - 1) // sy + 1, (F - 1) // sx + 1
    col = torch.empty(B * To * Fo, 9 * C, dtype=torch.bfloat16, device=A.device)
    check(_lib.lib().ea_im2col3x3(_p(A), _p(col), B, T, F, C, sy, sx, _stream()), "ea_im2col3x3")
    return col


def col2im3x3(dcol, B, T, F, C, sy, sx):
    dA = torch.empty(B * T * F, C, dtype=torch.bfloat16, device=dcol.device)
    check(_lib.lib().ea_col2im3x3(_p(dcol), _p(dA), B, T, F, C, sy, sx, _stream()), "ea_col2im3x3")
    return dA


def colstats(X, stats):
    M, C = X.shape
    check(_lib.lib().ea_colstats_bf16(_p(X), _p(stats), M, C, _stream()), "ea_colstats_bf16")
    return stats


def log_softmax(x, M, V, ld):
    out = torch.empty(M, V, dtype=torch.float32, device=x.device)
    if x.dtype == torch.float32:
        check(_lib.lib().ea_log_softmax_f32(_p(x), ld, _p(out), M, V, _stream()), "ea_log_softmax_f32")
    else:
        assert x.dtype == torch.bfloat16
        check(_lib.lib().ea_log_softmax_bf16(_p(x), ld, _p(out), M, V, _stream()), "ea_log_softmax_bf16")
    return out


def ctc_loss_fwd(lprobs, targets, in_len, tgt_len, B, T, V, Lmax, blank):
    assert lprobs.dtype == torch.float32 and lprobs.is_contiguous()
    assert targets.dtype == torch.int32 and in_len.dtype == torch.int32 and tgt_len.dtype == torch.int32
    dev = lprobs.device
    nll = torch.empty(B, dtype=torch.float32, device=dev)
    ws = torch.empty(int(_lib.lib().ea_ctc_workspace_bytes(B, T, Lmax)), dtype=torch.uint8, device=dev)
    check(
        _lib.lib().ea_ctc_loss(_p(lprobs), _p(targets), _p(in_len), _p(tgt_len), _p(nll), _p(ws), B, T, V, Lmax, blank,
                               _stream()),
        "ea_ctc_loss",
    )
    return nll, ws


def ctc_loss_grad(lprobs, ws, nll, targets, in_len, tgt_len, B, T, V, Lmax, blank, ld_out=None, grad_bf16=True,
                  grad_scale=1.0, grad_scale_dev=None, zero_infinity=True):
    ld_out = V if ld_out is None else ld_out
    dl = torch.empty(B * T, ld_out, dtype=torch.bfloat16 if grad_bf16 else torch.float32, device=lprobs.device)
    check(
        _lib.lib().ea_ctc_grad(_p(lprobs), _p(ws), _p(nll), _p(targets), _p(in_len), _p(tgt_len), _p(dl), ld_out,
                               int(grad_bf16), B, T, V, Lmax, blank, grad_scale, _p(grad_scale_dev),
                               int(zero_infinity), _stream()),
        "ea_ctc_grad",
    )
    return dl


SMOOTHING = {"uniform": 0, "unigram": 1, "temporal": 2}


def label_smoothed_ce(logits, ld, target, M, V, pad_idx, eps, want_grad=True, grad_bf16=True, grad_scale=1.0,
                      grad_ld=None, smoothing="uniform", prior=None, tgt_len=0):
    assert target.dtype == torch.int32
    dev = logits.device
    out = torch.zeros(2, dtype=torch.float32, device=dev)
    dl = None
    grad_ld = V if grad_ld is None else grad_ld
    if want_grad:
        dl = torch.zeros(M, grad_ld, dtype=torch.bfloat16 if grad_bf16 else torch.float32, device=dev)
    check(
        _lib.lib().ea_label_smoothed_ce(_p(logits), ld, int(logits.dtype == torch.bfloat16), _p(target), _p(out),
                                        _p(dl), grad_ld, int(grad_bf16), M, V, pad_idx, eps, grad_scale, SMOOTHING[smoothing],
                                        _p(prior), tgt_len, _stream()),
        "ea_label_smoothed_ce",
    )
    return out, dl


def fbank_batch(wav, offsets, B, tables, cmvn_mean, cmvn_std, Tmax, nmel=80, frame_len=400, frame_shift=160,
                preemph=0.97, log_floor=1.1920928955078125e-07, want_sum=True):
    dev = wav.device
    feat = torch.empty(B, Tmax, nmel, dtype=torch.float32, device=dev)
    utt_sum = torch.zeros(B, dtype=torch.float32, device=dev) if want_sum else None
    out_len = torch.empty(B, dtype=torch.int32, device=dev)
    assert wav.dtype in (torch.float32, torch.int16)
    fn = _lib.lib().ea_fbank_batch if wav.dtype == torch.float32 else _lib.lib().ea_fbank_batch_i16
    check(
        fn(_p(wav), _p(offsets), B, _p(tables["window"]), _p(tables["twiddle"]), _p(tables["mel_start"]), _p(tables["mel_len"]),
           _p(tables["mel_woff"]), _p(tables["mel_w"]), _p(cmvn_mean), _p(cmvn_std), _p(feat), _p(utt_sum), _p(out_len), Tmax, nmel,
           frame_len, frame_shift, preemph, log_floor, _stream()),
        "ea_fbank_batch",
    )
    return feat, out_len, utt_sum


def feature_stats(feat, lengths, acc):
    B, Tmax, nmel = feat.shape
    assert acc.dtype == torch.float64 and acc.numel() == 2 * nmel + 1 and feat.dtype == torch.float32 and feat.is_contiguous()
    check(_lib.lib().ea_feature_stats(_p(feat), _p(lengths), _p(acc), B, Tmax, nmel, _stream()), "ea_feature_stats")
    return acc


def specaugment(feat, lengths, utt_sum, fmask, tmask, use_mean=True, mask_value=0.0):
    B, Tmax, nmel = feat.shape
    nf = fmask.shape[1] if fmask is not None else 0
    nt = tmask.shape[1] if tmask is not None else 0
    check(
        _lib.lib().ea_specaugment(_p(feat), _p(lengths), _p(utt_sum), _p(fmask), _p(tmask), nf, nt, B, Tmax, nmel,
                                  int(use_mean), mask_value, _stream()),
        "ea_specaugment",
    )
    return feat


def grad_sumsq(g, out):
    check(_lib.lib().ea_grad_sumsq(_p(g), g.numel(), _p(out), _stream()), "ea_grad_sumsq")
    return out


def clip_coef(sumsq, pre_scale, max_norm, coef, denom_dev=None):
    check(_lib.lib().ea_clip_coef(_p(sumsq), pre_scale, _p(denom_dev), max_norm, _p(coef), _stream()), "ea_clip_coef")
    return coef


def adam_step(p, g, m, v, p_bf16, coef, lr, beta1, beta2, eps, weight_decay, step, zero_grad=True):
    check(
        _lib.lib().ea_adam_step(_p(p), _p(g), _p(m), _p(v), _p(p_bf16), p.numel(), _p(coef), lr, beta1, beta2, eps,
                                weight_decay, step, int(zero_grad), _stream()),
        "ea_adam_step",
    )


def ctc_greedy_decode(x, in_len, B, T, V, blank, pad, ld=None, want_align=True):
    dev = x.device
    ld = x.stride(0) if ld is None else ld
    best = torch.empty(B * T, dtype=torch.int32, device=dev)
    bestv = torch.empty(B * T, dtype=torch.float32, device=dev)
    tokens = torch.empty(B, T, dtype=torch.int32, device=dev)
    align = torch.zeros(B, T, dtype=torch.int32, device=dev) if want_align else None
    out_len = torch.empty(B, dtype=torch.int32, device=dev)
    score = torch.empty(B, dtype=torch.float32, device=dev)
    check(
        _lib.lib().ea_ctc_greedy_decode(_p(x), ld, int(x.dtype == torch.bfloat16), _p(in_len), _p(best), _p(bestv), _p(tokens),
                                        _p(align), _p(out_len), _p(score), B, T, V, blank, pad, _stream()),
        "ea_ctc_greedy_decode",
    )
    return tokens, out_len, score, align


# ... 591 lines not shown
```

include/espresso_amd.h:

```cpp
#ifndef ESPRESSO_AMD_H
#define ESPRESSO_AMD_H

#include <stdint.h>

#ifdef __cplusplus
extern "C" {
#endif

typedef struct ihipStream_t* ea_stream_t;

int ea_version(void);

enum { EA_ACT_NONE = 0, EA_ACT_RELU = 1, EA_ACT_SILU = 2 };

typedef struct EaGemmParams {
  const void* A;
  const void* B;
  void* C;
  void* C2;
  const float* bias;
  const void* resid;
  const void* aux;
  int M, N, K, batch, zdiv;
  int a_kstrided, b_kstrided, c_f32, accumulate, resid_f32, act;
  long lda, ldb, ldc, ldc2, ldr, ldaux;
  long sA_hi, sA_lo, sB_hi, sB_lo, sC_hi, sC_lo, sR_hi, sR_lo, sX_hi, sX_lo;
  float alpha, out_scale;
  uint64_t drop_seed;
  uint32_t drop_thr;
  float drop_scale;
  int splitk, kchunk;
  void* workspace;
  void* q_u;
  void* q_v;
  const float* pos_u;
  const float* pos_v;
  long ld_q;
  int qsplit_n;
  float qscale;
} EaGemmParams;

int ea_gemm_bf16(const EaGemmParams* p, ea_stream_t stream);
long ea_gemm_splitk_workspace_bytes(int M, int N, int batch, int splitk);
int ea_set_gemm_variant(int v);
int ea_set_gemm_xcd_swizzle(int mask);
int ea_set_gemm_glds(int stages);
long ea_set_gemm_nt_store_min_bytes(long bytes);
int ea_set_gemm_w8(int mode);
int ea_gemm_profile_enable(int on);
long ea_gemm_profile_read(double* total_ms, double* total_flops);
int ea_gemm_profile_bytes(double* total_bytes);
long ea_gemm_profile_dump(const char* path);

#define EA_WGRAD_MAX 16
typedef struct EaWgradProblem {
  const void* dy;
  const void* x;
  float* dW;
  float* dbias;
  int M, N, K;
  long ld_dy, ld_x, ldw;
} EaWgradProblem;
typedef struct EaWgradGroup {
  int count;
  EaWgradProblem p[EA_WGRAD_MAX];
} EaWgradGroup;
int ea_wgrad_group(const EaWgradGroup* group, ea_stream_t stream);
int ea_set_wgrad_transposing_reads(int on);
int ea_set_wgrad_w8(int mode);

int ea_layernorm_fwd(const void* x, const float* gamma, const float* beta, void* y, float* mean, float* rstd,
                     int M, int C, float eps, const uint8_t* row_zero, uint64_t drop_seed, uint32_t drop_thr,
                     float drop_scale, ea_stream_t stream);
int ea_layernorm_fwd_f32out(const void* x, const float* gamma, const float* beta, float* y, float* mean, float* rstd,
                            int M, int C, float eps, const uint8_t* row_zero, uint64_t drop_seed, uint32_t drop_thr,
                            float drop_scale, ea_stream_t stream);
int ea_layernorm_bwd_f32dy(const void* x, const float* dy, const float* gamma, const float* mean, const float* rstd,
                           void* dx, float* dgamma, float* dbeta, int M, int C, const uint8_t* row_zero,
                           uint64_t drop_seed, uint32_t drop_thr, float drop_scale, const void* dx_add,
                           void* workspace, ea_stream_t stream);
long ea_layernorm_bwd_workspace_bytes(int M, int C);
int ea_layernorm_bwd(const void* x, const void* dy, const float* gamma, const float* mean, const float* rstd,
                     void* dx, float* dgamma, float* dbeta, int M, int C, const uint8_t* row_zero,
                     uint64_t drop_seed, uint32_t drop_thr, float drop_scale, const void* dx_add,
                     void* workspace, ea_stream_t stream);
int ea_layernorm_bwd_dx(const void* x, const void* dy, const float* gamma, const float* mean, const float* rstd, void* dx,
                        float* dgamma, float* dbeta, int M, int C, const uint8_t* row_zero, uint64_t drop_seed,
                        uint32_t drop_thr, float drop_scale, const void* dx_add, void* workspace, ea_stream_t stream);
int ea_layernorm_param_reduce(const void* workspace, float* dgamma, float* dbeta, int M, int C, ea_stream_t stream);
#define EA_LNRED_MAX 8
typedef struct EaLnReduceItem { const void* workspace; float* dgamma; float* dbeta; int M, C; } EaLnReduceItem;
typedef struct EaLnReduceGroup { int count; EaLnReduceItem item[EA_LNRED_MAX]; } EaLnReduceGroup;
int ea_layernorm_param_reduce_group(const EaLnReduceGroup* group, ea_stream_t stream);
int ea_layernorm_bwd_dx2(const void* x, const void* dy, const float* gamma, const float* mean, const float* rstd, void* dx,
                         float* dgamma, float* dbeta, int M, int C, const void* dx_add, void* workspace, void* out2, float a2,
                         uint64_t seed2, uint32_t thr2, float scale2, ea_stream_t stream);
int ea_layernorm_fwd2(const void* x, const float* g1, const float* b1, void* y1, float* mean1, float* rstd1, const float* g2,
                      const float* b2, void* y2, float* mean2, float* rstd2, int M, int C, float eps, ea_stream_t stream);
int ea_layernorm_bwd2_dx(const void* x1, const void* dy1, const float* gamma1, const float* mean1, const float* rstd1,
                         const void* dx_add, void* ws1, const void* x2, const float* gamma2, const float* mean2, const float* rstd2,
                         void* ws2, void* dx, int M, int C, void* out2, float a2, uint64_t seed2, uint32_t thr2, float scale2,
                         ea_stream_t stream);

int ea_cast_f32_to_bf16(const float* src, void* dst, long n, ea_stream_t stream);
int ea_transpose_bf16_batch(const void* const* src, void* const* dst, const int* rows, const int* cols, int n, ea_stream_t stream);
int ea_audio_probe(const char* path, long* num_samples, int* sample_rate, int* channels, int* bits);
long ea_audio_read_i16(const char* path, int16_t* dst, long capacity, int* sample_rate);
int ea_audio_verify(const char* path);
int ea_audio_read_batch_i16(const char* const* paths, int n, int16_t* dst, const long* offsets, int num_threads, long* lengths,
                            int* sample_rates);

int ea_cast_f32_to_bf16_rows(const float* src, long ld_src, void* dst, long ld_dst, long M, int N, ea_stream_t stream);
int ea_cast_bf16_to_f32(const void* src, float* dst, long n, ea_stream_t stream);
int ea_scale_dropout_bf16(const void* x, const void* y, void* out, long n, float a, float b, uint64_t seed,
                          uint32_t thr, float inv_keep, ea_stream_t stream);
int ea_colsum_bf16(const void* X, float* out, int M, int N, long ld, ea_stream_t stream);
int ea_embedding_fwd(const int* tokens, const int* positions, const float* W, const float* pos_table, void* out, int M,
                     int C, float scale, ea_stream_t stream);
int ea_embedding_bwd(const int* tokens, const void* dy, float* dW, int M, int C, float scale, int pad_idx,
                     ea_stream_t stream);
int ea_zero_rows_bf16(void* x, const uint8_t* row_zero, int M, int C, ea_stream_t stream);

int ea_flash_attention_supported(int dh, int T, int S, int relpos);
int ea_flash_attention_fwd(const void* qu, const void* qv, long ldq, const void* k, const void* v, long ldkv,
                           const void* pp, long ldpp, const int* key_len, void* out, long ldo, float* lse, int H, int B,
                           int T, int S, int dh, int causal, uint64_t drop_seed, uint32_t drop_thr, float drop_scale,
                           void* keep_bits, ea_stream_t stream);
long ea_flash_keep_bits_bytes(int H, int B, int T);
int ea_set_flash_relpos(int on);
int ea_flash_keep_bits(void* keep_bits, int H, int B, int T, uint64_t drop_seed, uint32_t drop_thr, ea_stream_t stream);
int ea_flash_attention_bwd(const void* qu, const void* qv, long ldq, const void* k, const void* v, long ldkv,
                           const void* pp, long ldpp, const int* key_len, const void* out, const void* dout, long ldo,
                           const float* lse, float* D, void* t1, void* t2, long ldt, void* dBD, int ld_bd, void* dk,
                           void* dv, long lddkv, int H, int B, int T, int S, int dh, int causal, float scaling,
                           uint64_t drop_seed, uint32_t drop_thr, float drop_scale, const void* keep_bits,
                           void* dq, long lddq, ea_stream_t stream);

int ea_relpos_q_prep(const void* qkv, long ldq, const float* u, const float* v, void* qu, void* qv, int M,
                     int C, float scaling, ea_stream_t stream);
int ea_relpos_softmax_fwd(const float* ac, const float* bd, const int* key_len, const float* attn_mask, void* P,
                          void* Pd, int H, int B, int T, int S, int ld_ac, int ld_bd, int ld_p, int causal,
                          uint64_t drop_seed, uint32_t drop_thr, float drop_scale, ea_stream_t stream);
int ea_relpos_softmax_bwd(const void* P, const float* dPd, void* dAC, void* dBD, int H, int B, int T, int S,
                          int ld_p, int ld_dp, int ld_bd, uint64_t drop_seed, uint32_t drop_thr,
                          float drop_scale, ea_stream_t stream);
int ea_add2_strided_bf16(const void* a, long lda, const void* b, long ldb, void* out, long ldo, int M, int C,
                         ea_stream_t stream);

int ea_glu_dwconv_fwd(const void* Y, const float* w, void* U, void* Z, double* stats, int B, int T, int C, int KW,
                      ea_stream_t stream);
int ea_bn_finalize(const double* stats, float* mean_rstd, float* running_mean, float* running_var, int C, float n,
                   float eps, float momentum, ea_stream_t stream);
int ea_bn_from_running(const float* running_mean, const float* running_var, float* mean_rstd, int C, float eps,
                       ea_stream_t stream);
int ea_bn_act_fwd(const void* Z, const float* mean_rstd, const float* gamma, const float* beta, void* H, long M,
                  int C, int act, ea_stream_t stream);
int ea_bn_act_bwd(const void* Z, const void* dH, const float* mean_rstd, const float* gamma, const float* beta,
                  float* red, void* dZ, float* dgamma, float* dbeta, long M, int C, int act, int training,
                  ea_stream_t stream);
long ea_dwconv_wgrad_workspace_bytes(int B, int T, int C, int KW);
int ea_glu_dwconv_bwd(const void* dZ, const void* Y, const void* U, const float* w, void* dY, float* dw,
                      void* wgrad_ws, int B, int T, int C, int KW, ea_stream_t stream);
int ea_dwconv_bwd_weight(const void* dZ, const void* U, float* dw, void* wgrad_ws, int B, int T, int C, int KW, ea_stream_t stream);
int ea_bn_act_fwd_train(const void* Z, const double* stats, float* mean_rstd, float* running_mean, float* running_var,
                        const float* gamma, const float* beta, void* H, long M, int C, int act, float n, float eps,
                        float momentum, double* zero_next, int zero_n, ea_stream_t stream);
int ea_bn_act_bwd_fused(const void* Z, const void* dH, const float* mean_rstd, const float* gamma, const float* beta,
                        float* red, void* dZ, float* dgamma, float* dbeta, long M, int C, int act, int training,
                        float* zero_next, int zero_n, ea_stream_t stream);
int ea_bn_glu_dwconv_bwd_fused(const void* Z, const void* dH, const float* mean_rstd, const float* gamma, const float* beta, float* red,
                               void* dZ, float* dgamma, float* dbeta, int act, int training, float* zero_next, int zero_n,
                               const void* Y, const float* w, void* dY, int B, int T, int C, int KW, ea_stream_t stream);
int ea_bn_param_grad(const float* red, float* dgamma, float* dbeta, int C, ea_stream_t stream);
int ea_conv1_bn_bwd(const float* X, const void* Z, const void* dH, const float* mean_rstd, const float* gamma, const float* beta,
                    float* red, float* dgamma, float* dbeta, float* dW, float* dbias, int B, int T, int F, int CO, int sy, int sx,
                    int act, int training, ea_stream_t stream);

int ea_conv1_fwd(const float* X, const float* W, const float* bias, void* Z, double* stats, int B, int T, int F,
                 int CO, int sy, int sx, ea_stream_t stream);
int ea_conv1_wgrad(const float* X, const void* dZ, float* dW, float* dbias, int B, int T, int F, int CO, int sy,
                   int sx, ea_stream_t stream);
int ea_conv3x3_fwd(const void* X, const void* W, const float* bias, void* Z, double* stats, int B, int T, int F, int Cin,
                   int Cout, int sy, int sx, ea_stream_t stream);
int ea_conv3x3_dgrad(const void* dZ, const void* Wd, void* dX, int B, int T, int F, int Cin, int Cout, int sy, int sx,
                     ea_stream_t stream);
long ea_conv3x3_wgrad_workspace_bytes(int B, int T, int F, int Cin, int Cout, int sy, int sx);
int ea_conv3x3_wgrad(const void* X, const void* dZ, float* dW, void* workspace, int B, int T, int F, int Cin, int Cout, int sy,
                     int sx, ea_stream_t stream);
int ea_conv3x3_wgrad_param_layout(const void* X, const void* dZ, float* dW, void* workspace, int B, int T, int F, int Cin, int Cout,
                                  int sy, int sx, ea_stream_t stream);
int ea_im2col3x3(const void* A, void* col, int B, int T, int F, int C, int sy, int sx, ea_stream_t stream);
int ea_col2im3x3(const void* dcol, void* dA, int B, int T, int F, int C, int sy, int sx, ea_stream_t stream);
int ea_colstats_bf16(const void* X, double* stats, long M, int C, ea_stream_t stream);

int ea_log_softmax_f32(const float* in, long ld_in, float* out, long M, int V, ea_stream_t stream);
int ea_log_softmax_bf16(const void* in, long ld_in, float* out, long M, int V, ea_stream_t stream);
long ea_ctc_workspace_bytes(int B, int T, int Lmax);
int ea_ctc_loss(const float* lprobs, const int* targets, const int* in_len, const int* tgt_len, float* nll,
                void* workspace, int B, int T, int V, int Lmax, int blank, ea_stream_t stream);
int ea_ctc_grad(const float* lprobs, const void* workspace, const float* nll, const int* targets,
                const int* in_len, const int* tgt_len, void* dlogits, long ld_out, int dlogits_bf16, int B, int T,
                int V, int Lmax, int blank, float grad_scale, const float* grad_scale_dev, int zero_infinity,
                ea_stream_t stream);
int ea_ctc_greedy_decode(const void* x, long ld, int x_bf16, const int* in_len, int* best, float* bestv, int* tokens,
                         int* align, int* out_len, float* score, int B, int T, int V, int blank, int pad,
                         ea_stream_t stream);
long ea_ctc_prefix_beam_workspace_bytes(int B, int T, int beam);
int ea_ctc_prefix_beam_step(const void* x, long ld, int x_bf16, const int* in_len, void* workspace, const float* lm_rows,
                            long ld_lm, int* lm_parent, int* lm_token, void* lm_keep, int B, int T, int V, int beam, int K,
                            int blank, float lm_weight, float ins_bonus, int t0, int t1, ea_stream_t stream);
int ea_ctc_prefix_beam_finish(void* workspace, const float* lm_rows, long ld_lm, float lm_weight, float ins_bonus, int eos,
                              int B, int T, int beam, int nbest, int pad, int* tokens, int* lengths, float* scores, int* nhyp,
                              ea_stream_t stream);
long ea_ctc_prefix_beam_bias_workspace_bytes(int B, int T, int beam);
int ea_ctc_prefix_beam_bias_step(const void* x, long ld, int x_bf16, const int* in_len, void* workspace, const float* lm_rows,
                                 long ld_lm, int* lm_parent, int* lm_token, void* lm_keep, const int* cg_nodes,
                                 const int* cg_edges, const int* cg_root, int cg_n_nodes, int cg_n_edges, int B, int T, int V,
                                 int beam, int K, int blank, float lm_weight, float ins_bonus, int t0, int t1, ea_stream_t stream);
int ea_ctc_prefix_beam_bias_finish(void* workspace, const float* lm_rows, long ld_lm, float lm_weight, float ins_bonus, int eos,
                                   const int* cg_nodes, int cg_n_nodes, int B, int T, int beam, int nbest, int pad, int* tokens,
                                   int* lengths, float* scores, int* nhyp, ea_stream_t stream);
int ea_context_graph_score_host(const int* nodes_host, const int* edges_host, const int* root_host, int n_nodes, int n_edges,
                                int V, const int* tokens_host, const int* lens_host, int N, int L, float* running_host,
                                float* final_host, int* q_host);
int ea_context_graph_score(const int* nodes, const int* edges, const int* root, int n_nodes, int n_edges, int V,
                           const int* tokens, const int* lens, int N, int L, float* running, float* final_bias, int* q_out,
                           ea_stream_t stream);
long ea_rnnt_frame_beam_workspace_bytes(int B, int T, int beam);
int ea_rnnt_frame_beam_step(const float* logits, long ld, const float* lm_rows, long ld_lm, int lm_no_blank, const int* in_len,
                            void* workspace, int* parent, int* token, void* keep, int B, int T, int V, int beam, int K, int blank,
                            int eos, float temperature, float lm_weight, int t, ea_stream_t stream);
int ea_rnnt_frame_beam_finish(void* workspace, int B, int T, int beam, int nbest, int pad, int normalize, int* tokens,
                              int* lengths, float* scores, int* nhyp, ea_stream_t stream);
long ea_rnnt_frame_beam_stream_state_bytes(int max_frames, int beam);
int ea_rnnt_frame_beam_stream_reset(void* state, const int* slots, int n, int max_streams, int max_frames, int beam,
                                    ea_stream_t stream);
int ea_rnnt_frame_beam_stream_step(const float* logits, long ld, const float* lm_rows, long ld_lm, int lm_no_blank,
                                   const int* slot_idx, const int* n_new, int j, int n, void* state, int* parent, int* token,
                                   void* keep, int max_streams, int max_frames, int V, int beam, int K, int blank, int eos,
                                   float temperature, float lm_weight, ea_stream_t stream);
int ea_rnnt_frame_beam_stream_finish(const void* state, const int* slots, int n, int max_streams, int max_frames, int beam,
                                     int nbest, int pad, int normalize, int max_u, int* tokens, int* lengths, float* scores,
                                     int* nhyp, ea_stream_t stream);
int ea_rnnt_frame_beam_stream_partial(const void* state, const int* slots, int n, int max_streams, int max_frames, int beam,
                                      int pad, int max_u, int* tokens, int* lengths, float* scores, int* stable_len,
                                      ea_stream_t stream);
int ea_ngram_create(const char* path, void* handle_host, char* err_host, long err_cap);
int ea_ngram_destroy(void* handle);
int ea_ngram_info(const void* handle, int* meta_host, long* counts_host);
long ea_ngram_vocab(const void* handle, char* buf_host, long cap);
long ea_ngram_records(const void* handle, int order, int* ngrams_host, float* logp_host, float* bow_host);
int ea_ngram_upload(void* handle);
int ea_ngram_score_host(const void* handle, const int* ctx_host, const int* words_host, int N, float* out_host);
int ea_ngram_score(const void* handle, const int* ctx, const int* words, int N, float* out, ea_stream_t stream);
long ea_ctc_lexicon_beam_workspace_bytes(int B, int T, int beam);
int ea_ctc_lexicon_beam_search(const void* x, long ld, int x_bf16, const int* in_len, void* workspace, const void* ngram,
                               const int* trie_off, const int* trie_tok, const int* trie_child, const int* trie_word,
                               const float* trie_smear, const void* word_start, int space, int B, int T, int V, int beam, int K,
                               int blank, float lm_weight, float word_score, float ins_bonus, int nbest, int pad, int* tokens,
                               int* lengths, float* scores, int* nhyp, ea_stream_t stream);
long ea_ctc_lexicon_stream_state_bytes(int max_frames, int beam);
int ea_ctc_lexicon_stream_reset(void* state, const int* slots, int n, const void* ngram, int max_streams, int max_frames,
                                int beam, ea_stream_t stream);
int ea_ctc_lexicon_stream_step(const void* x, long ld, int x_bf16, long total_rows, const int* slot_idx, const int* n_new,
                               const int* row_off, int n, void* state, const void* ngram, const int* trie_off,
                               const int* trie_tok, const int* trie_child, const int* trie_word, const float* trie_smear,
                               const void* word_start, int space, int max_streams, int max_frames, int V, int beam, int K,
                               int blank, float lm_weight, float word_score, float ins_bonus, ea_stream_t stream);
int ea_ctc_lexicon_stream_finish(const void* state, const int* slots, int n, const void* ngram, const int* trie_word,
                                 const float* trie_smear, int max_streams, int max_frames, int beam, float lm_weight,
                                 float word_score, float ins_bonus, int nbest, int pad, int max_u, int* tokens, int* lengths,
                                 float* scores, int* nhyp, ea_stream_t stream);
int ea_ctc_lexicon_stream_partial(const void* state, const int* slots, int n, int max_streams, int max_frames, int beam,
                                  float ins_bonus, int pad, int max_u, int* tokens, int* lengths, float* scores, int* stable_len,
                                  ea_stream_t stream);
int ea_label_smoothed_ce(const void* logits, long ld, int logits_bf16, const int* target, float* out_loss,
                         void* dlogits, long ld_out, int dlogits_bf16, long M, int V, int pad_idx, float eps,
                         float grad_scale, int smoothing, const float* prior, int tgt_len, ea_stream_t stream);

int ea_fbank_batch(const float* wav, const long* offsets, int B, const float* window, const float* twiddle,
                   const int* mel_start, const int* mel_len, const int* mel_woff, const float* mel_w,
                   const float* cmvn_mean, const float* cmvn_std, float* feat, float* utt_sum, int* out_len,
                   int Tmax, int nmel, int frame_len, int frame_shift, float preemph, float log_floor,
                   ea_stream_t stream);
int ea_fbank_batch_i16(const int16_t* wav, const long* offsets, int B, const float* window, const float* twiddle,
                   const int* mel_start, const int* mel_len, const int* mel_woff, const float* mel_w,
                   const float* cmvn_mean, const float* cmvn_std, float* feat, float* utt_sum, int* out_len,
                   int Tmax, int nmel, int frame_len, int frame_shift, float preemph, float log_floor,
                   ea_stream_t stream);
int ea_specaugment(float* feat, const int* lengths, const float* utt_sum, const int* fmask, const int* tmask,
                   int nf, int nt, int B, int Tmax, int nmel, int use_mean, float mask_value, ea_stream_t stream);

int ea_feature_stats(const float* feat, const int* lengths, double* acc, int B, int Tmax, int nmel, ea_stream_t stream);

int ea_grad_sumsq(const float* g, long n, float* out, ea_stream_t stream);
int ea_clip_coef(const float* sumsq, float pre_scale, const float* denom_dev, float max_norm, float* coef,
                 ea_stream_t stream);
int ea_adam_step(float* p, float* g, float* m, float* v, void* p_bf16, long n, const float* coef, float lr,
                 float beta1, float beta2, float eps, float weight_decay, int step, int zero_grad,
                 ea_stream_t stream);

typedef struct EaFfnParams { const float *ln_g, *ln_b; const void* w1; const float* b1; const void* w2; const float* b2; } EaFfnParams;
typedef struct EaFfnGrads { float *ln_g, *ln_b, *w1, *b1, *w2, *b2; } EaFfnGrads;
typedef struct EaAttnParams {
  const float *ln_g, *ln_b; const void* wqkv; const float* bqkv; const void* wo; const float* bo;
  const float *pos_u, *pos_v; const void* wpos;
} EaAttnParams;
typedef struct EaAttnGrads { float *ln_g, *ln_b, *wqkv, *bqkv, *wo, *bo, *pos_u, *pos_v, *wpos; } EaAttnGrads;
typedef struct EaConvParams {
  const float *ln_g, *ln_b; const void* pw1; const float* dw; const float *bn_g, *bn_b; float *bn_rm, *bn_rv; const void* pw2;
} EaConvParams;
typedef struct EaConvGrads { float *ln_g, *ln_b, *pw1, *dw, *bn_g, *bn_b, *pw2; } EaConvGrads;
typedef struct EaLayerGrads { EaFfnGrads ffn1; EaAttnGrads attn; EaConvGrads conv; EaFfnGrads ffn2; float *final_ln_g, *final_ln_b; } EaLayerGrads;
typedef struct EaConformerLayer {
  EaFfnParams ffn1; EaAttnParams attn; EaConvParams conv; EaFfnParams ffn2; const float *final_ln_g, *final_ln_b;
  EaLayerGrads grads;
  void* wt;
} EaConformerLayer;
typedef struct EaLayerShape {
  int B, T, C, H, F, KW, training; float p_drop, p_act, p_attn; uint64_t seed; int has_attn_mask;
  int scratch_clean;
  int pos_mode, act;
  int S;
  int defer;
  int wt_fresh;
} EaLayerShape;

enum {
  EA_SITE_FFN1_ACT = 0, EA_SITE_FFN1_OUT = 1, EA_SITE_ATTN_PROBS = 2, EA_SITE_ATTN_OUT = 3, EA_SITE_CONV_OUT = 4,
  EA_SITE_FFN2_ACT = 5, EA_SITE_FFN2_OUT = 6, EA_SITE_CROSS_PROBS = 7, EA_SITE_CROSS_OUT = 8
};
uint64_t ea_layer_dropout_seed(uint64_t layer_seed, int site);
int ea_dropout_hash_host(uint64_t seed, uint64_t idx0, long n, uint32_t* out);

int ea_set_backward_overlap(int on);
int ea_set_backward_deferred(int on);
int ea_set_backward_deferred_inline(int on);
int ea_backward_flush(ea_stream_t stream);
int ea_streams_share_queue(ea_stream_t a, ea_stream_t b);
int ea_side_stream_report(int* rejected, int* unprobed);
int ea_conformer_layer_workspace(const EaLayerShape* shape, long* saved_bytes, long* scratch_bytes);
int ea_conformer_layer_refresh_wt(const EaConformerLayer* layer, const EaLayerShape* shape, ea_stream_t stream);
int ea_conformer_layer_fwd(const EaConformerLayer* layer, const EaLayerShape* shape, const void* x_in, void* x_out,
// ... 142 lines not shown
```

Before: 5.315 audio-hours/sec.

## Fuse BN affine and ReLU into next conv3x3 input load in forward and wgrad

Adds a bn_finalize_affine kernel that folds BatchNorm into a per-channel scale and shift. The next implicit-GEMM conv3x3 forward and its wgrad kernel then apply scale, shift and ReLU to the raw pre-BN activation while loading operands, with padding taps masked per row. This removes the separate bn_act_fwd pass and the materialized activation tensor between subsampling conv layers. In exchange it adds per-fragment ALU work and extra LDS inside the GEMM inner loops, which may cost occupancy or MFMA throughput.

```diff
diff --git a/espresso_amd/csrc/conv_igemm.hip b/espresso_amd/csrc/conv_igemm.hip
--- a/espresso_amd/csrc/conv_igemm.hip
+++ b/espresso_amd/csrc/conv_igemm.hip
@@ -22,9 +22,17 @@
   int N;
   long ldw;
   int OT, OF, ot_mul, ot_add, of_mul, of_add;
+  const float* xscale;
+  const float* xshift;
 };
 
-template <int BN_>
+__device__ __forceinline__ uint32_t xf_relu_bf2(uint32_t w, float sc_lo, float sh_lo, float sc_hi, float sh_hi) {
+  const float lo = __uint_as_float(w << 16), hi = __uint_as_float(w & 0xffff0000u);
+  const float ylo = lo * sc_lo + sh_lo, yhi = hi * sc_hi + sh_hi;
+  return pack_bf2(fmaxf(ylo, 0.f), fmaxf(yhi, 0.f));
+}
+
+template <int BN_, bool XF = false>
 __global__ __launch_bounds__(256, 2) void conv_gather_kernel(const ConvGatherArgs a) {
   constexpr int BM_ = 128, NST = 2;
   constexpr int NJ = BN_ / 32;
@@ -95,12 +103,54 @@
   }
 
   if (nk > 0) issue(0, 0);
+  float* xss = reinterpret_cast<float*>(dsm + NST * STAGE);
+  uint32_t xvalid[4];
+  float xsc[2][8], xsh[2][8];
+  auto xf_load = [&](int chunk) {
+#pragma unroll
+    for (int ks = 0; ks < 2; ++ks) {
+      const float* ps = xss + chunk * BK + (ks * 4 + (lane >> 4)) * 8;
+      const float4 s0 = *reinterpret_cast<const float4*>(ps), s1 = *reinterpret_cast<const float4*>(ps + 4);
+      const float4 h0 = *reinterpret_cast<const float4*>(ps + a.SC), h1 = *reinterpret_cast<const float4*>(ps + a.SC + 4);
+      xsc[ks][0] = s0.x; xsc[ks][1] = s0.y; xsc[ks][2] = s0.z; xsc[ks][3] = s0.w;
+      xsc[ks][4] = s1.x; xsc[ks][5] = s1.y; xsc[ks][6] = s1.z; xsc[ks][7] = s1.w;
+      xsh[ks][0] = h0.x; xsh[ks][1] = h0.y; xsh[ks][2] = h0.z; xsh[ks][3] = h0.w;
+      xsh[ks][4] = h1.x; xsh[ks][5] = h1.y; xsh[ks][6] = h1.z; xsh[ks][7] = h1.w;
+    }
+  };
+  if constexpr (XF) {
+    for (int c = tid; c < a.SC; c += 256) {
+      xss[c] = a.xscale[c];
+      xss[a.SC + c] = a.xshift[c];
+    }
+#pragma unroll
+    for (int i = 0; i < 4; ++i) {
+      const uint32_t p = m0 + wm * 64 + i * 16 + (lane & 15);
+      xvalid[i] = 0;
+      if (p < M) {
+        const uint32_t q = p / (uint32_t)a.RF, b = q / (uint32_t)a.RT;
+        const int rf = (int)(p - q * a.RF) * a.af, rt = (int)(q - b * a.RT) * a.at;
+#pragma unroll 1
+        for (int t = 0; t < a.ntaps; ++t)
+          if ((unsigned)(rt + a.bt[t]) < (unsigned)a.ST && (unsigned)(rf + a.bf[t]) < (unsigned)a.SF) xvalid[i] |= 1u << t;
+      }
+    }
+    __syncthreads();
+    xf_load(0);
+  }
   int stage = 0;
   for (int kt = 0; kt < nk; ++kt) {
     asm volatile("s_waitcnt vmcnt(0)" ::: "memory");
     __builtin_amdgcn_s_barrier();
     if (kt + 1 < nk) issue(stage ^ 1, kt + 1);
     const char* st = dsm + stage * STAGE;
+    uint32_t xkeep[4];
+    if constexpr (XF) {
+      const int tap = kt / cpt;
+      if (cpt > 1) xf_load(kt - tap * cpt);
+#pragma unroll
+      for (int i = 0; i < 4; ++i) xkeep[i] = 0u - ((xvalid[i] >> tap) & 1u);
+    }
 #pragma unroll
     for (int ks = 0; ks < 2; ++ks) {
       bf16x8_t af[4], bfr[NJ];
@@ -108,6 +158,17 @@
       for (int i = 0; i < 4; ++i) af[i] = *reinterpret_cast<const bf16x8_t*>(st + a_off[ks][i]);
 #pragma unroll
       for (int j = 0; j < NJ; ++j) bfr[j] = *reinterpret_cast<const bf16x8_t*>(st + b_off[ks][j]);
+      if constexpr (XF) {
+#pragma unroll
+        for (int i = 0; i < 4; ++i) {
+          uint4 u = __builtin_bit_cast(uint4, af[i]);
+          u.x = xf_relu_bf2(u.x, xsc[ks][0], xsh[ks][0], xsc[ks][1], xsh[ks][1]) & xkeep[i];
+          u.y = xf_relu_bf2(u.y, xsc[ks][2], xsh[ks][2], xsc[ks][3], xsh[ks][3]) & xkeep[i];
+          u.z = xf_relu_bf2(u.z, xsc[ks][4], xsh[ks][4], xsc[ks][5], xsh[ks][5]) & xkeep[i];
+          u.w = xf_relu_bf2(u.w, xsc[ks][6], xsh[ks][6], xsc[ks][7], xsh[ks][7]) & xkeep[i];
+          af[i] = __builtin_bit_cast(bf16x8_t, u);
+        }
+      }
 #pragma unroll
       for (int i = 0; i < 4; ++i)
 #pragma unroll
@@ -197,16 +258,17 @@
   return z;
 }
 
-template <int BN_>
+template <int BN_, bool XF = false>
 int launch_gather(const ConvGatherArgs& a, hipStream_t stream) {
-  constexpr int bytes = 2 * (128 + BN_) * ROW_BYTES;
-  static bool attr_ok = hipFuncSetAttribute(reinterpret_cast<const void*>(&conv_gather_kernel<BN_>),
+  constexpr int bytes = 2 * (128 + BN_) * ROW_BYTES + (XF ? 2 * 128 * (int)sizeof(float) : 0);
+  static bool attr_ok = hipFuncSetAttribute(reinterpret_cast<const void*>(&conv_gather_kernel<BN_, XF>),
                                             hipFuncAttributeMaxDynamicSharedMemorySize, bytes) == hipSuccess;
   if (!attr_ok) return -1;
+  if (XF && (a.SC > 128 || !a.xscale || !a.xshift)) return -2;
   const long M = (long)a.RB * a.RT * a.RF;
   if (M <= 0) return 0;
   if (M >= (1L << 31) - 128) return -1;
-  hipLaunchKernelGGL((conv_gather_kernel<BN_>), dim3((unsigned)((M + 127) / 128)), dim3(256), bytes, stream, a);
+  hipLaunchKernelGGL((conv_gather_kernel<BN_, XF>), dim3((unsigned)((M + 127) / 128)), dim3(256), bytes, stream, a);
   return EA_CHECK_LAUNCH();
 }
 
@@ -221,6 +283,8 @@
   int bt[9], bf[9];
   int chunks_per_wg;
   int ablate;
+  const float* xscale;
+  const float* xshift;
 };
 
 __device__ __forceinline__ int tr_sw(int r) { return (r & 3) ^ ((r >> 3) & 1); }
@@ -234,7 +298,7 @@
       : "memory");
 }
 
-template <int DEPTH, int NT>
+template <int DEPTH, int NT, bool XF = false>
 __global__ __launch_bounds__(256, NT == 9 ? 2 : 4) void conv_wgrad_kernel(const ConvWgradArgs a) {
   constexpr int TILE = 64 * ROW_BYTES;
   constexpr int NBUF = DEPTH == 1 ? 2 : 4;
@@ -242,6 +306,7 @@
   const int tap0 = NT == 9 ? 0 : (int)(blockIdx.z % 3) * 3;
   const int zsplit = NT == 9 ? (int)blockIdx.z : (int)(blockIdx.z / 3);
   __shared__ __attribute__((aligned(16))) char lds[(2 + NBUF) * TILE];
+  __shared__ __attribute__((aligned(16))) uint16_t xrow[XF ? 2 : 1][64];
   const int tid = threadIdx.x, lane = tid & 63, wave = tid >> 6;
   const int wr = wave >> 1, wc = wave & 1;
   const int co0 = blockIdx.x * 64, ci0 = blockIdx.y * 64;
@@ -267,6 +332,10 @@
   }
   int rowb[2], rowt[2], rowf[2];
   long rowp[2];
+  auto tap_ok = [&](int i, int tap) {
+    const int st = rowt[i] + a.bt[tap0 + tap], sf = rowf[i] + a.bf[tap0 + tap];
+    return rowb[i] >= 0 && (unsigned)st < (unsigned)a.ST && (unsigned)sf < (unsigned)a.SF;
+  };
   auto decode = [&](long ch) {
 #pragma unroll
     for (int i = 0; i < 2; ++i) {
@@ -281,6 +350,12 @@
         rowb[i] = -1;
         rowt[i] = rowf[i] = 0;
       }
+      if constexpr (XF) {
+        uint32_t m = 0;
+#pragma unroll
+        for (int t = 0; t < NT; ++t) m |= tap_ok(i, t) ? 1u << t : 0u;
+        if ((lane & 7) == 0) xrow[ch & 1][rr[i]] = (uint16_t)m;
+      }
     }
   };
   auto issue_A = [&](int abuf) {
@@ -299,6 +374,15 @@
       __builtin_amdgcn_global_load_lds((gptr_t)s, (lptr_t)(lds + (2 + buf) * TILE + (wave + 4 * i) * 1024), 16, 0, 0);
     }
   };
+  float xsc[2], xsh[2];
+  uint32_t xm[2][4];
+  if constexpr (XF) {
+#pragma unroll
+    for (int t = 0; t < 2; ++t) {
+      xsc[t] = a.xscale[ci0 + wc * 32 + t * 16 + (lane & 15)];
+      xsh[t] = a.xshift[ci0 + wc * 32 + t * 16 + (lane & 15)];
+    }
+  }
   const uint32_t lds0 = (uint32_t)(uintptr_t)lds;
   auto read_frags = [&](int tile_off, int c0, uint4 (&fr)[2][2]) {
     const int g = lane >> 4, i = lane & 15;
@@ -351,6 +435,7 @@
     else if (pend == 4) asm volatile("s_waitcnt vmcnt(4)" ::: "memory");
     else if (pend == 2) asm volatile("s_waitcnt vmcnt(2)" ::: "memory");
     else asm volatile("s_waitcnt vmcnt(0)" ::: "memory");
+    if constexpr (XF) asm volatile("s_waitcnt lgkmcnt(0)" ::: "memory");
     if (!(a.ablate & 8)) __builtin_amdgcn_s_barrier();
     uint4 fb[2][2];
     if (!(a.ablate & 4) || s == 0) {
@@ -358,6 +443,32 @@
       read_frags((2 + (s & (NBUF - 1))) * TILE, wc * 32, fb);
     } else {
       fb[0][0] = fb[0][1] = fb[1][0] = fb[1][1] = fa[0][0];
+    }
+    if constexpr (XF) {
+      if (tap == 0) {
+#pragma unroll
+        for (int ks = 0; ks < 2; ++ks) {
+          const uint4 m = *reinterpret_cast<const uint4*>(&xrow[ch & 1][ks * 32 + 8 * (lane >> 4)]);
+          xm[ks][0] = m.x; xm[ks][1] = m.y; xm[ks][2] = m.z; xm[ks][3] = m.w;
+        }
+      }
+#pragma unroll
+      for (int ks = 0; ks < 2; ++ks) {
+        uint32_t keep[4];
+#pragma unroll
+        for (int e = 0; e < 4; ++e) {
+          const uint32_t b = (xm[ks][e] >> tap) & 0x00010001u;
+          keep[e] = (b << 16) - b;
+        }
+#pragma unroll
+        for (int t = 0; t < 2; ++t) {
+          uint4& u = fb[ks][t];
+          u.x = xf_relu_bf2(u.x, xsc[t], xsh[t], xsc[t], xsh[t]) & keep[0];
+          u.y = xf_relu_bf2(u.y, xsc[t], xsh[t], xsc[t], xsh[t]) & keep[1];
+          u.z = xf_relu_bf2(u.z, xsc[t], xsh[t], xsc[t], xsh[t]) & keep[2];
+          u.w = xf_relu_bf2(u.w, xsc[t], xsh[t], xsc[t], xsh[t]) & keep[3];
+        }
+      }
     }
     __builtin_amdgcn_sched_barrier(0);
     issue_next();
@@ -445,12 +556,13 @@
 
 }
 
-extern "C" int ea_conv3x3_fwd(const void* X, const void* W, const float* bias, void* Z, double* stats, int B, int T, int F,
-                              int Cin, int Cout, int sy, int sx, hipStream_t stream) {
+static int conv3x3_fwd_impl(const void* X, const float* xscale, const float* xshift, const void* W, const float* bias, void* Z,
+                            double* stats, int B, int T, int F, int Cin, int Cout, int sy, int sx, hipStream_t stream) {
   if (B <= 0 || T <= 0 || F <= 0) return 0;
   if (Cin % 64 || (Cout != 64 && Cout != 128) || sy < 1 || sx < 1) return -2;
   ConvGatherArgs a;
   a.src = (const bf16_t*)X; a.W = (const bf16_t*)W; a.out = (bf16_t*)Z; a.bias = bias; a.stats = stats;
+  a.xscale = xscale; a.xshift = xshift;
   a.zero = zero_line(stream);
   if (!a.zero) return -1;
   const int To = (T - 1) / sy + 1, Fo = (F - 1) / sx + 1;
@@ -465,7 +577,18 @@
     }
   a.N = Cout; a.ldw = 9L * Cin;
   a.OT = To; a.OF = Fo; a.ot_mul = 1; a.ot_add = 0; a.of_mul = 1; a.of_add = 0;
+  if (xscale) return Cout == 128 ? launch_gather<128, true>(a, stream) : launch_gather<64, true>(a, stream);
   return Cout == 128 ? launch_gather<128>(a, stream) : launch_gather<64>(a, stream);
+}
+extern "C" int ea_conv3x3_fwd(const void* X, const void* W, const float* bias, void* Z, double* stats, int B, int T, int F,
+                              int Cin, int Cout, int sy, int sx, hipStream_t stream) {
+  return conv3x3_fwd_impl(X, nullptr, nullptr, W, bias, Z, stats, B, T, F, Cin, Cout, sy, sx, stream);
+}
+extern "C" int ea_conv3x3_fwd_bnrelu(const void* X, const float* xscale, const float* xshift, const void* W, const float* bias,
+                                     void* Z, double* stats, int B, int T, int F, int Cin, int Cout, int sy, int sx,
+                                     hipStream_t stream) {
+  if (!xscale || !xshift || Cin > 128) return -2;
+  return conv3x3_fwd_impl(X, xscale, xshift, W, bias, Z, stats, B, T, F, Cin, Cout, sy, sx, stream);
 }
 
 extern "C" int ea_conv3x3_dgrad(const void* dZ, const void* Wd, void* dX, int B, int T, int F, int Cin, int Cout, int sy, int sx,
@@ -479,6 +602,7 @@
     for (int pf = 0; pf < sx; ++pf) {
       ConvGatherArgs a;
       a.src = (const bf16_t*)dZ; a.W = (const bf16_t*)Wd; a.out = (bf16_t*)dX; a.bias = nullptr; a.stats = nullptr; a.zero = zero;
+      a.xscale = a.xshift = nullptr;
       a.RB = B; a.RT = (T - pt + sy - 1) / sy; a.RF = (F - pf + sx - 1) / sx;
       a.ST = To; a.SF = Fo; a.SC = Cout;
       a.at = 1; a.af = 1;
@@ -506,22 +630,31 @@
   return (long)wgrad_split((long)B * To * Fo, Cin, Cout) * Cout * 9 * Cin * (long)sizeof(float);
 }
 
-static int conv3x3_wgrad_impl(const void* X, const void* dZ, float* dW, void* workspace, int B, int T, int F, int Cin, int Cout,
-                              int sy, int sx, int param_layout, hipStream_t stream);
+static int conv3x3_wgrad_impl(const void* X, const float* xscale, const float* xshift, const void* dZ, float* dW, void* workspace,
+                              int B, int T, int F, int Cin, int Cout, int sy, int sx, int param_layout, int taps_arg,
+                              hipStream_t stream);
 extern "C" int ea_conv3x3_wgrad(const void* X, const void* dZ, float* dW, void* workspace, int B, int T, int F, int Cin, int Cout,
                                 int sy, int sx, hipStream_t stream) {
-  return conv3x3_wgrad_impl(X, dZ, dW, workspace, B, T, F, Cin, Cout, sy, sx, 0, stream);
+  return conv3x3_wgrad_impl(X, nullptr, nullptr, dZ, dW, workspace, B, T, F, Cin, Cout, sy, sx, 0, 0, stream);
 }
 extern "C" int ea_conv3x3_wgrad_param_layout(const void* X, const void* dZ, float* dW, void* workspace, int B, int T, int F, int Cin,
                                              int Cout, int sy, int sx, hipStream_t stream) {
-  return conv3x3_wgrad_impl(X, dZ, dW, workspace, B, T, F, Cin, Cout, sy, sx, 1, stream);
-}
-static int conv3x3_wgrad_impl(const void* X, const void* dZ, float* dW, void* workspace, int B, int T, int F, int Cin, int Cout,
-                              int sy, int sx, int param_layout, hipStream_t stream) {
+  return conv3x3_wgrad_impl(X, nullptr, nullptr, dZ, dW, workspace, B, T, F, Cin, Cout, sy, sx, 1, 0, stream);
+}
+extern "C" int ea_conv3x3_wgrad_bnrelu(const void* X, const float* xscale, const float* xshift, const void* dZ, float* dW,
+                                       void* workspace, int B, int T, int F, int Cin, int Cout, int sy, int sx, int param_layout,
+                                       int taps, hipStream_t stream) {
+  if (!xscale || !xshift || (taps != 0 && taps != 3 && taps != 9)) return -2;
+  return conv3x3_wgrad_impl(X, xscale, xshift, dZ, dW, workspace, B, T, F, Cin, Cout, sy, sx, param_layout, taps, stream);
+}
+static int conv3x3_wgrad_impl(const void* X, const float* xscale, const float* xshift, const void* dZ, float* dW, void* workspace,
+                              int B, int T, int F, int Cin, int Cout, int sy, int sx, int param_layout, int taps_arg,
+                              hipStream_t stream) {
   if (B <= 0 || T <= 0 || F <= 0) return 0;
   if (Cin % 64 || Cout % 64 || sy < 1 || sx < 1 || !workspace) return -2;
   ConvWgradArgs a;
   a.X = (const bf16_t*)X; a.dZ = (const bf16_t*)dZ; a.slab = (float*)workspace;
+  a.xscale = xscale; a.xshift = xshift;
   a.zero = zero_line(stream);
   if (!a.zero) return -1;
   const int To = (T - 1) / sy + 1, Fo = (F - 1) / sx + 1;
@@ -539,8 +672,11 @@
   static const int depth_env = [] { const char* e = getenv("EA_CONV_WGRAD_DEPTH"); return e ? atoi(e) : 0; }();
   const int depth = depth_env ? depth_env : (Cout <= 64 ? 3 : 1);
   static const int taps_env = [] { const char* e = getenv("EA_CONV_WGRAD_TAPS"); return e ? atoi(e) : 0; }();
-  const int taps = taps_env == 3 || taps_env == 9 ? taps_env : 3;
-  if (taps == 3) {
+  const int taps = taps_arg ? taps_arg : (taps_env == 3 || taps_env == 9 ? taps_env : 3);
+  if (xscale) {
+    if (taps == 3) hipLaunchKernelGGL((conv_wgrad_kernel<1, 3, true>), dim3(Cout / 64, Cin / 64, nsplit * 3), dim3(256), 0, stream, a);
+    else hipLaunchKernelGGL((conv_wgrad_kernel<1, 9, true>), dim3(Cout / 64, Cin / 64, nsplit), dim3(256), 0, stream, a);
+  } else if (taps == 3) {
     hipLaunchKernelGGL((conv_wgrad_kernel<1, 3>), dim3(Cout / 64, Cin / 64, nsplit * 3), dim3(256), 0, stream, a);
   } else if (depth == 1) hipLaunchKernelGGL((conv_wgrad_kernel<1, 9>), dim3(Cout / 64, Cin / 64, nsplit), dim3(256), 0, stream, a);
   else if (depth == 2) hipLaunchKernelGGL((conv_wgrad_kernel<2, 9>), dim3(Cout / 64, Cin / 64, nsplit), dim3(256), 0, stream, a);
diff --git a/espresso_amd/csrc/convmodule.hip b/espresso_amd/csrc/convmodule.hip
--- a/espresso_amd/csrc/convmodule.hip
+++ b/espresso_amd/csrc/convmodule.hip
@@ -195,6 +195,32 @@
   if (c >= C) return;
   mean_rstd[c] = running_mean[c];
   mean_rstd[C + c] = rsqrtf(running_var[c] + eps);
+}
+
+__global__ void bn_finalize_affine_kernel(const double* __restrict__ stats, float* __restrict__ mean_rstd,
+                                          float* __restrict__ running_mean, float* __restrict__ running_var,
+                                          const float* __restrict__ gamma, const float* __restrict__ beta,
+                                          float* __restrict__ scale_shift, int C, float n, float eps, float momentum) {
+  const int c = blockIdx.x * blockDim.x + threadIdx.x;
+  if (c >= C) return;
+  if (stats) {
+    const float mean = (float)(stats[c] / (double)n);
+    float var = (float)(stats[C + c] / (double)n - (stats[c] / (double)n) * (stats[c] / (double)n));
+    var = fmaxf(var, 0.f);
+    mean_rstd[c] = mean;
+    mean_rstd[C + c] = rsqrtf(var + eps);
+    if (running_mean) {
+      running_mean[c] = (1.f - momentum) * running_mean[c] + momentum * mean;
+      const float unb = n > 1.f ? var * n / (n - 1.f) : var;
+      running_var[c] = (1.f - momentum) * running_var[c] + momentum * unb;
+    }
+  } else {
+    mean_rstd[c] = running_mean[c];
+    mean_rstd[C + c] = rsqrtf(running_var[c] + eps);
+  }
+  const float sc = mean_rstd[C + c] * gamma[c];
+  scale_shift[c] = sc;
+  scale_shift[C + c] = beta[c] - mean_rstd[c] * sc;
 }
 
 __global__ __launch_bounds__(256) void bn_act_fwd_kernel(const bf16_t* __restrict__ Z, const float* __restrict__ mean_rstd,
@@ -734,6 +760,14 @@
                      mean_rstd, C, eps);
   return EA_CHECK_LAUNCH();
 }
+extern "C" int ea_bn_finalize_affine(const double* stats, float* mean_rstd, float* running_mean, float* running_var,
+                                     const float* gamma, const float* beta, float* scale_shift, int C, float n, float eps,
+                                     float momentum, hipStream_t stream) {
+  if (!stats && (!running_mean || !running_var)) return -2;
+  hipLaunchKernelGGL(bn_finalize_affine_kernel, dim3((C + 255) / 256), dim3(256), 0, stream, stats, mean_rstd, running_mean,
+                     running_var, gamma, beta, scale_shift, C, n, eps, momentum);
+  return EA_CHECK_LAUNCH();
+}
 extern "C" int ea_bn_act_fwd(const void* Z, const float* mean_rstd, const float* gamma, const float* beta, void* H,
                              long M, int C, int act, hipStream_t stream) {
   if (M <= 0) return 0;
diff --git a/espresso_amd/functional.py b/espresso_amd/functional.py
--- a/espresso_amd/functional.py
+++ b/espresso_amd/functional.py
@@ -679,6 +679,15 @@
     return old
 
 
+_CONV_FUSED_BNRELU = True
+
+
+def set_conv_fused_bn_relu(on: bool) -> bool:
+    global _CONV_FUSED_BNRELU
+    old, _CONV_FUSED_BNRELU = _CONV_FUSED_BNRELU, bool(on)
+    return old
+
+
 def set_conv_implicit_gemm(on: bool):
     global _CONV_IGEMM
     _CONV_IGEMM = bool(on)
@@ -697,6 +706,8 @@
         saved = []
         cfgs = []
         A = None
+        Aff = None
+        chans = [1] + [params[4 * j].shape[0] for j in range(L)]
         Tc, Fc, Cc = T, F, 1
         for i in range(L):
             w, b, g, beta = params[4 * i: 4 * i + 4]
@@ -711,7 +722,7 @@
                 col, w16 = None, None
             elif _conv_igemm_ok(Cc, Co, sy, sx):
                 w16 = K.cast_f32_to_bf16(w.detach().permute(0, 2, 3, 1).reshape(Co, 9 * Cc).contiguous())
-                Zi = K.conv3x3_fwd(A, w16, b, B, Tc, Fc, Cc, Co, sy, sx, stats=stats)
+                Zi = K.conv3x3_fwd(A, w16, b, B, Tc, Fc, Cc, Co, sy, sx, stats=stats, in_scale_shift=Aff)
                 col = A
             else:
                 col = K.im2col3x3(A, B, Tc, Fc, Cc, sy, sx)
@@ -721,9 +732,14 @@
                 if training:
                     K.colstats(Zi, stats)
             n = B * To * Fo
-            mr = K.bn_finalize(stats, Co, n, bn_eps, bn_momentum, rm, rv) if training else K.bn_from_running(rm, rv, bn_eps)
-            A = K.bn_act_fwd(Zi, mr, g, beta, "relu")
-            saved += [Zi, mr, col, w16, g, beta]
+            in_aff = Aff if col is not None else None
+            if _CONV_FUSED_BNRELU and i + 1 < L and _conv_igemm_ok(Co, chans[i + 2], *strides[i + 1]):
+                mr, Aff = K.bn_finalize_affine(stats, g, beta, Co, n, bn_eps, bn_momentum, rm, rv)
+                A = Zi
+            else:
+                mr = K.bn_finalize(stats, Co, n, bn_eps, bn_momentum, rm, rv) if training else K.bn_from_running(rm, rv, bn_eps)
+                A, Aff = K.bn_act_fwd(Zi, mr, g, beta, "relu"), None
+            saved += [Zi, mr, col, w16, g, beta, in_aff]
             cfgs.append((Tc, Fc, Cc, To, Fo, Co, sy, sx))
             Tc, Fc, Cc = To, Fo, Co
         out = A.view(B * Tc, Fc * Cc)
@@ -733,7 +749,7 @@
         if row_zero is not None:
             K.zero_rows(out, row_zero)
         ctx.save_for_backward(X, row_zero, *[t for t in saved if t is not None])
-        ctx.layout = [[t is not None for t in saved[6 * i: 6 * i + 6]] for i in range(L)]
+        ctx.layout = [[t is not None for t in saved[7 * i: 7 * i + 7]] for i in range(L)]
         ctx.cfg = (B, cfgs, p_drop, seed, training, [tuple(p.shape) for p in params[0::4]])
         ctx.igemm = [i > 0 and _conv_igemm_ok(cfgs[i][2], cfgs[i][5], cfgs[i][6], cfgs[i][7]) for i in range(L)]
         ctx.weights = [params[4 * i] for i in range(L)]
@@ -763,7 +779,7 @@
         side = _side_stream(X.device)
         keep = []
         for i in range(L - 1, -1, -1):
-            Zi, mr, col, w16, g, beta = per[i]
+            Zi, mr, col, w16, g, beta, in_aff = per[i]
             Tc, Fc, Cc, To, Fo, Co, sy, sx = cfgs[i]
             pw, pb, pg, pbe = ctx.params[4 * i: 4 * i + 4]
             sg, sbe = (_grad_sink(pg, Co), _grad_sink(pbe, Co)) if training else (None, None)
@@ -800,11 +816,11 @@
                 side.wait_stream(cur)
                 if sW is not None:
                     with torch.cuda.stream(side):
-                        K.conv3x3_wgrad(col, dZ, sW, B, Tc, Fc, Cc, Co, sy, sx, param_layout=True)
+                        K.conv3x3_wgrad(col, dZ, sW, B, Tc, Fc, Cc, Co, sy, sx, param_layout=True, in_scale_shift=in_aff)
                 else:
                     dWp = _zeros_f32(Co * 9 * Cc, X).view(Co, 9 * Cc)
                     with torch.cuda.stream(side):
-                        K.conv3x3_wgrad(col, dZ, dWp, B, Tc, Fc, Cc, Co, sy, sx)
+                        K.conv3x3_wgrad(col, dZ, dWp, B, Tc, Fc, Cc, Co, sy, sx, in_scale_shift=in_aff)
                     grads[4 * i] = dWp.view(Co, 3, 3, Cc).permute(0, 3, 1, 2)
                 if not training:
                     db = g.detach() * mr[1] * dbeta
diff --git a/espresso_amd/kernels.py b/espresso_amd/kernels.py
--- a/espresso_amd/kernels.py
+++ b/espresso_amd/kernels.py
@@ -300,6 +300,14 @@
     return mean_rstd
 
 
+def bn_finalize_affine(stats, gamma, beta, C, n, eps, momentum, running_mean, running_var):
+    mean_rstd = torch.empty(2, C, dtype=torch.float32, device=gamma.device)
+    scale_shift = torch.empty(2, C, dtype=torch.float32, device=gamma.device)
+    check(_lib.lib().ea_bn_finalize_affine(_p(stats), _p(mean_rstd), _p(running_mean), _p(running_var), _p(gamma), _p(beta),
+                                           _p(scale_shift), C, float(n), eps, momentum, _stream()), "ea_bn_finalize_affine")
+    return mean_rstd, scale_shift
+
+
 def bn_act_fwd(Z, mean_rstd, gamma, beta, act):
     M, C = Z.shape
     H = torch.empty_like(Z)
@@ -350,9 +358,14 @@
     check(_lib.lib().ea_conv1_wgrad(_p(X), _p(dZ), _p(dW), _p(dbias), B, T, F, CO, sy, sx, _stream()), "ea_conv1_wgrad")
 
 
-def conv3x3_fwd(X, W16, bias, B, T, F, Cin, Cout, sy, sx, stats=None):
+def conv3x3_fwd(X, W16, bias, B, T, F, Cin, Cout, sy, sx, stats=None, in_scale_shift=None):
     To, Fo = (T - 1) // sy + 1, (F - 1) // sx + 1
     Z = torch.empty((B * To * Fo, Cout), dtype=torch.bfloat16, device=X.device)
+    if in_scale_shift is not None:
+        assert in_scale_shift.shape == (2, Cin) and in_scale_shift.dtype == torch.float32 and in_scale_shift.is_contiguous()
+        check(_lib.lib().ea_conv3x3_fwd_bnrelu(_p(X), _p(in_scale_shift[0]), _p(in_scale_shift[1]), _p(W16), _p(bias), _p(Z), _p(stats),
+                                               B, T, F, Cin, Cout, sy, sx, _stream()), "ea_conv3x3_fwd_bnrelu")
+        return Z
     check(_lib.lib().ea_conv3x3_fwd(_p(X), _p(W16), _p(bias), _p(Z), _p(stats), B, T, F, Cin, Cout, sy, sx, _stream()), "ea_conv3x3_fwd")
     return Z
 
@@ -363,10 +376,15 @@
     return dX
 
 
-def conv3x3_wgrad(X, dZ, dW, B, T, F, Cin, Cout, sy, sx, param_layout=False):
+def conv3x3_wgrad(X, dZ, dW, B, T, F, Cin, Cout, sy, sx, param_layout=False, in_scale_shift=None, taps=0):
     lib = _lib.lib()
     nb = lib.ea_conv3x3_wgrad_workspace_bytes(B, T, F, Cin, Cout, sy, sx)
     ws = torch.empty(nb, dtype=torch.uint8, device=X.device)
+    if in_scale_shift is not None:
+        assert in_scale_shift.shape == (2, Cin) and in_scale_shift.dtype == torch.float32 and in_scale_shift.is_contiguous()
+        check(lib.ea_conv3x3_wgrad_bnrelu(_p(X), _p(in_scale_shift[0]), _p(in_scale_shift[1]), _p(dZ), _p(dW), _p(ws), B, T, F, Cin, Cout,
+                                          sy, sx, int(param_layout), int(taps), _stream()), "ea_conv3x3_wgrad_bnrelu")
+        return dW
     fn = lib.ea_conv3x3_wgrad_param_layout if param_layout else lib.ea_conv3x3_wgrad
     check(fn(_p(X), _p(dZ), _p(dW), _p(ws), B, T, F, Cin, Cout, sy, sx, _stream()), "ea_conv3x3_wgrad")
     return dW
diff --git a/include/espresso_amd.h b/include/espresso_amd.h
--- a/include/espresso_amd.h
+++ b/include/espresso_amd.h
@@ -155,6 +155,8 @@
                        ea_stream_t stream);
 int ea_bn_act_fwd(const void* Z, const float* mean_rstd, const float* gamma, const float* beta, void* H, long M,
                   int C, int act, ea_stream_t stream);
+int ea_bn_finalize_affine(const double* stats, float* mean_rstd, float* running_mean, float* running_var, const float* gamma,
+                          const float* beta, float* scale_shift, int C, float n, float eps, float momentum, ea_stream_t stream);
 int ea_bn_act_bwd(const void* Z, const void* dH, const float* mean_rstd, const float* gamma, const float* beta,
                   float* red, void* dZ, float* dgamma, float* dbeta, long M, int C, int act, int training,
                   ea_stream_t stream);
@@ -189,6 +191,10 @@
                      int sx, ea_stream_t stream);
 int ea_conv3x3_wgrad_param_layout(const void* X, const void* dZ, float* dW, void* workspace, int B, int T, int F, int Cin, int Cout,
                                   int sy, int sx, ea_stream_t stream);
+int ea_conv3x3_fwd_bnrelu(const void* X, const float* xscale, const float* xshift, const void* W, const float* bias, void* Z,
+                          double* stats, int B, int T, int F, int Cin, int Cout, int sy, int sx, ea_stream_t stream);
+int ea_conv3x3_wgrad_bnrelu(const void* X, const float* xscale, const float* xshift, const void* dZ, float* dW, void* workspace,
+                            int B, int T, int F, int Cin, int Cout, int sy, int sx, int param_layout, int taps, ea_stream_t stream);
 int ea_im2col3x3(const void* A, void* col, int B, int T, int F, int C, int sy, int sx, ea_stream_t stream);
 int ea_col2im3x3(const void* dcol, void* dA, int B, int T, int F, int C, int sy, int sx, ea_stream_t stream);
 int ea_colstats_bf16(const void* X, double* stats, long M, int C, ea_stream_t stream);
```

New measurement: 5.236 audio-hours/sec. -1.5%, worse.
